# fpthink/PDGN

Measured on AMD Instinct MI355X. Metric: generator+D step points/sec (B=35, 256->2048 pts), higher is better.
Workload: dtype f32; 1 GPU; PDGNet_v2 G+D iteration (models/PDGNet_v2.py:171-256), chair-shaped synthetic batch, per-GPU batch 35, 256->2048 pts, random-init weights; global_batch=35, parallelism=dp1, losses_finite=True, hipgraph=False, issue=list

## Files before the change

include/pdgn_hip.h:

```cpp
#ifndef PDGN_HIP_H
#define PDGN_HIP_H

#include <stdint.h>

#ifdef __cplusplus
extern "C" {
#endif

#define PDGN_ERR_INVALID (-1)
#define PDGN_KNN_MAX_NSAMPLE 200

typedef void *pdgn_stream_t;

#define PDGN_ABI_VERSION 34
int pdgn_abi_version(void);

int pdgn_knnquery(int b, int n, int m, int nsample, const float *xyz, const float *new_xyz,
                  int32_t *idx, float *dist2, pdgn_stream_t stream);

int pdgn_grouping_forward(int b, int c, int n, int m, int nsample, const float *points,
                          const int32_t *idx, float *out, pdgn_stream_t stream);

int pdgn_grouping_backward(int b, int c, int n, int m, int nsample, const float *grad_out,
                           const int32_t *idx, float *grad_points, pdgn_stream_t stream);

int pdgn_nearestneighbor(int b, int n, int m, const float *unknown, const float *known,
                         float *dist2, int32_t *idx, pdgn_stream_t stream);

int pdgn_interpolation_forward(int b, int c, int m, int n, const float *points,
                               const int32_t *idx, const float *weight, float *out,
                               pdgn_stream_t stream);

int pdgn_interpolation_backward(int b, int c, int n, int m, const float *grad_out,
                                const int32_t *idx, const float *weight, float *grad_points,
                                pdgn_stream_t stream);

int pdgn_nndistance(int b, int n, const float *xyz, int m, const float *xyz2, float *result,
                    int32_t *result_i, float *result2, int32_t *result2_i, pdgn_stream_t stream);

int pdgn_nndistance_grad(int b, int n, const float *xyz1, int m, const float *xyz2,
                         const float *grad_dist1, const int32_t *idx1, const float *grad_dist2,
                         const int32_t *idx2, float *grad_xyz1, float *grad_xyz2,
                         pdgn_stream_t stream);

int pdgn_approxmatch(int b, int n, int m, const float *xyz1, const float *xyz2, float *match,
                     float *temp, pdgn_stream_t stream);

int pdgn_matchcost(int b, int n, int m, const float *xyz1, const float *xyz2,
                   const float *match, float *out, pdgn_stream_t stream);

int pdgn_matchcost_grad(int b, int n, int m, const float *xyz1, const float *xyz2,
                        const float *match, float *grad1, float *grad2, pdgn_stream_t stream);

long long pdgn_emd_cost_temp_floats(long long pairs, int n, int m);
int pdgn_emd_cost(int b, int n, int m, const float *xyz1, const float *xyz2, float *temp,
                  float *out, pdgn_stream_t stream);

int pdgn_feature_knn(int b, int f, int n, int k, const float *x, float *sqnorm, int32_t *idx,
                     pdgn_stream_t stream);

int pdgn_window_gather_sum(int b, int n, int k, int ldy, int T, int P, int C, int off, int offc,
                           const float *Y, const int32_t *idx, const float *bias, int bias_bstride,
                           float *out, pdgn_stream_t stream);
int pdgn_window_gather_sum_stats(int b, int n, int k, int ldy, int T, int P, int C, int off, int offc,
                                 const float *Y, const int32_t *idx, const float *bias, int bias_bstride,
                                 float *out, float *scratch, pdgn_stream_t stream);

int pdgn_window_gather_sum_backward(int b, int n, int k, int ldy, int T, int P, int C, int off,
                                    int offc, const float *dout, const int32_t *idx, float *dY,
                                    pdgn_stream_t stream);

int pdgn_knn_graph_transpose(int b, int n, int k, const int32_t *idx, int32_t *rowptr, int32_t *edges,
                             int32_t *scratch, pdgn_stream_t stream);
int pdgn_window_gather_sum_backward_csr(int b, int n, int k, int ldy, int T, int P, int C, int off,
                                        int offc, const float *dout, const int32_t *rowptr,
                                        const int32_t *edges, float *dY, unsigned *max_out, int max_init, pdgn_stream_t stream);

long long pdgn_bn_scratch_floats(long long rows, int c);
int pdgn_bn_stats(long long rows, int c, float eps, float momentum, const float *x, const float *gamma,
                  const float *beta, const float *pre_bias, float *running_mean, float *running_var,
                  float *scratch, float *stats, pdgn_stream_t stream);
int pdgn_bn_eval_stats(int c, float eps, const float *gamma, const float *beta, const float *pre_bias,
                       const float *running_mean, const float *running_var, float *stats,
                       pdgn_stream_t stream);
int pdgn_bn_stats_from_partials(long long rows, int c, float eps, float momentum, const float *gamma,
                                const float *beta, const float *pre_bias, float *running_mean, float *running_var,
                                const float *scratch, float *stats, pdgn_stream_t stream);
int pdgn_bn_stats_from_gemm_partials(long long rows, int c, long long nparts, int block_rows, float eps, float momentum,
                                     const float *gamma, const float *beta, const float *pre_bias,
                                     float *running_mean, float *running_var, const float *partials,
                                     float *stats, double *scratch, pdgn_stream_t stream);
long long pdgn_bn_blocks_scratch_doubles(int c, long long nparts);
int pdgn_bn_act_forward(long long rows, int c, int act, const float *x, const float *stats,
                        const float *mul, float *y, int interleave_n, pdgn_stream_t stream);
int pdgn_bn_act_backward(long long rows, int c, int act, int training, const float *x,
                         const float *dy, const float *mul, const float *stats, float *scratch,
                         float *bsums, float *dx, float *dmul, int interleave_n, pdgn_stream_t stream);

long long pdgn_bn_maxpool_scratch_floats(int b, int c);
int pdgn_bn_act_maxpool(int b, int n, int c, int act, const float *x, const float *stats, float *scratch,
                        float *ymax, int32_t *yarg, pdgn_stream_t stream);
long long pdgn_bn_stats_maxpool_scratch_floats(int b, int c);
int pdgn_bn_stats_act_maxpool(int b, int n, int c, int act, float eps, float momentum, const float *x, const float *gamma,
                              const float *beta, const float *pre_bias, float *running_mean, float *running_var, float *scratch,
                              float *stats, float *ymax, int32_t *yarg, pdgn_stream_t stream);
int pdgn_bn_act_maxpool_backward(int b, int n, int c, int act, int training, const float *x,
                                 const float *dout, const int32_t *yarg, const float *stats,
                                 float *scratch, float *bsums, float *dx, pdgn_stream_t stream);
long long pdgn_dense_bn_maxpool_backward_scratch(int b, int c, int k);
int pdgn_dense_bn_maxpool_backward(int b, int n, int c, int k, int act, const float *x, const float *dout, const int32_t *yarg,
                                   const float *stats, const float *h, int ldh, const float *W, int ldw, float *scratch,
                                   float *dh, float *dW, int lddw, float *bsums, pdgn_stream_t stream);
long long pdgn_dense_bn_maxpool_input_grad_scratch(int b, int c, int k);
int pdgn_dense_bn_maxpool_input_grad(int b, int n, int c, int k, int act, const float *x, const float *dout,
                                     const int32_t *yarg, const float *stats, const float *h, int ldh,
                                     const float *W, int ldw, float *scratch, float *dh, pdgn_stream_t stream);

int pdgn_group_colsum(long long groups, long long group_rows, int c, const float *x, long long ldx, float *out,
                      pdgn_stream_t stream);

int pdgn_softmax_slots_permute(long long m, int k, int c, const float *h, float *w, pdgn_stream_t stream);
int pdgn_bn_softmax_slots_permute(long long m, int k, int c, int act, const float *x, const float *stats,
                                  float *w, pdgn_stream_t stream);
int pdgn_bn_softmax_slots_permute_mul(long long m, int k, int c, int act, const float *x, const float *stats,
                                      int act_u, const float *u, const float *stats_u, float *w, float *y,
                                      unsigned *max_out, const float *gamma_u, const float *beta_u, float bound_scale,
                                      unsigned *cmax_out, pdgn_stream_t stream);
long long pdgn_bilateral_scratch_floats(long long m, int k, int c);
int pdgn_bilateral_weighting_backward(long long m, int k, int c, int act, int training, const float *x,
                                      const float *stats_x, const float *u, const float *stats_u, const float *w,
                                      const float *dy, float *scratch, float *bsums_x, float *bsums_u, float *dx,
                                      float *du, pdgn_stream_t stream);
int pdgn_softmax_slots_permute_backward(long long m, int k, int c, const float *w, const float *dw,
                                        float *dh, pdgn_stream_t stream);

int pdgn_skinny_nt(int R, int N, int K, const float *A, int lda, const float *B, int ldb, const float *bias, float *C, int ldc,
                   pdgn_stream_t stream);
int pdgn_skinny_nn(int R, int N, int K, const float *A, int lda, const float *B, int ldb, float *C, int ldc, pdgn_stream_t stream);
int pdgn_skinny_nt_act(int R, int N, int K, const float *A, int lda, const float *B, int ldb, const float *bias, float *C, int ldc,
                       int act, pdgn_stream_t stream);
int pdgn_skinny_nn_masked(int R, int N, int K, const float *A, int lda, const float *P, int ldp, int act, const float *B,
                          int ldb, float *C, int ldc, pdgn_stream_t stream);
int pdgn_skinny_tn(int R, int N, int K, const float *A, int lda, const float *B, int ldb, float *C, int ldc, pdgn_stream_t stream);
int pdgn_split_bf16x3(int rows, int cols, const float *src, int ld_src, unsigned short *planes, int ld_planes,
                      long long plane_stride, unsigned short *planes_t, int ld_planes_t, long long plane_stride_t,
                      pdgn_stream_t stream);
int pdgn_gemm_nt_ps(long long m, int n, int k, const float *A, int lda, const unsigned short *Wplanes, int ldw, long long wplane,
                    int parts, const float *bias, const float *addend, int ldadd, float *C, int ldc, float *stat_part,
                    const float *row_bias, int ld_rb, int rows_per_group, int act, const float *gate, int ldgate,
                    pdgn_stream_t stream);
long long pdgn_gemm_tail_workspace_floats(long long m, int n, int k, int with_stats);
long long pdgn_gemm_tn_big_workspace_floats(long long m, int n, int k);
int pdgn_gemm_set_tail_workspace(float *ws, long long floats);
int pdgn_gemm_nt_ps_launch_info(long long m, int n, int k, int parts, const void **sym, int *grid);
int pdgn_gemm_aux_symbols(const void **reduce, const void **scan);
int pdgn_gemm_set_mode(int mode);
int pdgn_gemm_set_scale_slots(void *slots, long long bytes);
int pdgn_absmax_rows_cols(long long rows, int cols, const float *src, int ld, unsigned *rowmax, unsigned *colmax,
                          pdgn_stream_t stream);
int pdgn_gemm_set_operand_scales(const unsigned *max_a, const unsigned *max_w);
int pdgn_gemm_two_part(long long m, int n, int k, long long scan_bytes);
int pdgn_gemm_two_part_planes(long long m, int n, int k, long long scan_bytes);
long long pdgn_gemm_nt_ps_stat_rows(long long m, int n, int k, int parts, int plain);
int pdgn_gemm_nt_ps_stat_block_rows(long long m, int n, int k, int parts, int plain);
int pdgn_gemm_nt_ps_row_panel(long long m, int n, int k, int parts, int plain);
long long pdgn_gemm_nt_ps_workspace_floats(long long m, int n, int k, int parts, int with_stats);
int pdgn_split_f16x2(int rows, int cols, const float *src, int ld_src, unsigned short *planes, int ld_planes,
                     long long plane_stride, unsigned short *planes_t, int ld_planes_t, long long plane_stride_t,
                     pdgn_stream_t stream);
int pdgn_gemm_set_config(int cfg);
int pdgn_gemm_set_shape(int shape);
int pdgn_gemm_nt(long long m, int n, int k, const float *A, int lda, const float *W, int ldw,
                 const float *bias, const float *addend, int ldadd, float *C, int ldc, float *stat_part,
                 pdgn_stream_t stream);
long long pdgn_thin_stat_rows(long long m);
int pdgn_thin_stat_block_rows(void);
int pdgn_thin_nt(long long m, int n, int k, const float *X, int ldx, const float *W, int wrs, int wcs,
                 const float *bias, float *Y, int ldy, float *stat_part, pdgn_stream_t stream);
int pdgn_thin_nt_ex(long long m, int n, int k, const float *X, int ldx, const float *W, int wrs, int wcs,
                    const float *bias, float *Y, int ldy, float *stat_part, const float *gate, int ldgate, pdgn_stream_t stream);
int pdgn_thin_tn(long long m, int ta, int wb, const float *A, int lda, const float *B, int ldb, float *O, int osi,
                 int osj, float *sum_a, float *sum_b, pdgn_stream_t stream);
int pdgn_gemm_nn(long long m, int n, int k, const float *A, int lda, const float *Wt, int ldw,
                 const float *bias, const float *addend, int ldadd, float *C, int ldc, float *stat_part,
                 pdgn_stream_t stream);
int pdgn_gemm_tn_big(long long m, int n, int k, const float *dY, int ldy, const float *X, int ldx, float *dW, int dw_is_zero,
                     pdgn_stream_t stream);
int pdgn_gemm_nt_ex(long long m, int n, int k, const float *A, int lda, const float *W, int ldw, const float *bias,
                    const float *addend, int ldadd, float *C, int ldc, float *stat_part, const float *row_bias, int ld_rb,
                    int rows_per_group, int act, const float *gate, int ldgate, int transposed_w, pdgn_stream_t stream);
long long pdgn_gemm_nt_stat_rows(long long m, int n, int k);
int pdgn_gemm_nt_stat_block_rows(long long m, int n, int k);
int pdgn_gemm_nt_config(long long m, int n, int k, int with_stats);

int pdgn_gemm_tn(long long m, int n, int k, const float *dY, const float *X, float *dW,
                 pdgn_stream_t stream);

int pdgn_local_stats(int b, int n, int m, int k, const float *xyz, const int32_t *idx, float *mu,
                     float *cov, pdgn_stream_t stream);
int pdgn_local_stats_backward(int b, int n, int m, int k, const float *xyz, const int32_t *idx,
                              const float *dmu, const float *dcov, float *dxyz, pdgn_stream_t stream);

int pdgn_chamfer_gram(int b, int m, int n, int d, const float *x, const float *y, float *minx,
                      int32_t *argx, float *miny, int32_t *argy, pdgn_stream_t stream);
int pdgn_chamfer_gram_grad(int b, int m, int n, int d, const float *x, const float *y,
                           const float *gminx, const int32_t *argx, const float *gminy,
                           const int32_t *argy, float *gx, float *gy, pdgn_stream_t stream);
int pdgn_chamfer_gram_grad_uniform(int b, int m, int n, int d, const float *x, const float *y, const float *g,
                                   float scale, const int32_t *argx, const int32_t *argy, float *gx, float *gy,
                                   pdgn_stream_t stream);
int pdgn_scaled_sum(long long n, const float *x, float scale, float *out, pdgn_stream_t stream);
int pdgn_mse_const(long long n, const float *x, float target, float scale, float *out, pdgn_stream_t stream);
int pdgn_mse_const_backward(long long n, const float *x, float target, float scale, const float *g, float *dx,
                            pdgn_stream_t stream);

int pdgn_emd_cost_indexed(int npairs, int n, int m, const float *xyz1, const int32_t *ia,
                          const float *xyz2, const int32_t *ib, float *temp, float *out,
                          pdgn_stream_t stream);
int pdgn_chamfer_gram_indexed(int npairs, int m, int n, int d, const float *x, const int32_t *ia,
                              const float *y, const int32_t *ib, float *minx, int32_t *argx,
                              float *miny, int32_t *argy, pdgn_stream_t stream);

int pdgn_deconv_assemble(int F, int Fo, int k, int T, int fc, const float *Wi, const float *W2, const float *Wf,
                         float *WcatC, float *WcatV, float *Wb, pdgn_stream_t stream);
int pdgn_deconv_assemble_backward(int F, int Fo, int k, int T, int fc, const float *gWcatC, const float *gWcatV,
                                  const float *gWb, float *dWi, float *dW2, float *dWf, pdgn_stream_t stream);

int pdgn_sample_bias(int b, int ldy, int nspec, const int *T, const int *C, const int *off, const int *offc,
                     const float *const *bias, const float *Yc, float *bb, pdgn_stream_t stream);
int pdgn_sample_bias_backward(int b, int ldy, int nspec, const int *T, const int *C, const int *off, const int *offc,
                              const float *g, float *dYc, float *const *dbias, pdgn_stream_t stream);

int pdgn_small_mlp_forward(int r, int k, int n, int act, int bn_mode, float eps, float momentum, const float *x,
                           const float *W, const float *bias, const float *gamma, const float *beta,
                           float *running_mean, float *running_var, float *y, float *pre, float *stat,
                           pdgn_stream_t stream);
int pdgn_small_mlp_backward(int r, int k, int n, int act, int bn_mode, const float *x, const float *dy, const float *pre,
                            const float *stat, const float *gamma, const float *beta, float *dpre, float *dgamma,
                            float *dbeta, float *dbias, float *dW, pdgn_stream_t stream);

int pdgn_ballquery(int b, int n, int m, float radius, int nsample, const float *new_xyz, const float *xyz,
                   int32_t *idx, pdgn_stream_t stream);
int pdgn_furthestsampling(int b, int n, int m, const float *xyz, float *temp, int32_t *idx, pdgn_stream_t stream);
int pdgn_gathering_forward(int b, int c, int n, int m, const float *points, const int32_t *idx, float *out,
                           pdgn_stream_t stream);
int pdgn_gathering_backward(int b, int c, int n, int m, const float *grad_out, const int32_t *idx,
                            float *grad_points, pdgn_stream_t stream);
int pdgn_grouping_int_forward(int b, int c, int n, int m, int nsample, const long long *points, const int32_t *idx,
                              long long *out, pdgn_stream_t stream);
int pdgn_featuredistribute(int b, int n, int m, const float *max_xyz, const float *xyz, int32_t *distribute_idx,
                           pdgn_stream_t stream);
int pdgn_labelstat_idx(int b, int n, int m, int nsample, int nclass, const int32_t *label_stat, const int32_t *idx,
                       int32_t *new_label_stat, pdgn_stream_t stream);
int pdgn_labelstat_ballrange(int b, int n, int m, float radius, int nclass, const float *new_xyz, const float *xyz,
                             const int32_t *label_stat, int32_t *new_label_stat, pdgn_stream_t stream);
int pdgn_labelstat_and_ballquery(int b, int n, int m, float radius, int nsample, int nclass, const float *new_xyz,
                                 const float *xyz, const int32_t *label_stat, int32_t *idx, int32_t *new_label_stat,
                                 pdgn_stream_t stream);

long long pdgn_point_max_scratch(int b, int n, int c);
int pdgn_point_max(int b, int n, int c, const float *x, float *scratch_val, int32_t *scratch_arg, float *out, int32_t *arg,
                   pdgn_stream_t stream);
int pdgn_point_max_backward(int b, int n, int c, const float *grad_out, const int32_t *arg, float *grad_x,
                            pdgn_stream_t stream);

int pdgn_spin(unsigned int microseconds, pdgn_stream_t stream);

int pdgn_replay_marker(int id, pdgn_stream_t stream);
int pdgn_replay_build(void *hip_graph, void **plan_out);
int pdgn_replay_info(void *plan, int *counts8);
int pdgn_replay_chains(void *plan, int *labels, int *nodes_per_chain);
int pdgn_replay_set_stream(void *plan, int chain, pdgn_stream_t stream);
int pdgn_replay_launch(void *plan);
int pdgn_replay_launch_range(void *plan, int lo, int hi);
int pdgn_replay_position(void *plan, int chain, int nth);
int pdgn_replay_points(void *plan, int *ids, int *pos, int *chain, int max_out);
int pdgn_replay_joined(void *plan);
int pdgn_replay_kernel_nodes(void *plan, const void *sym, int gx, int *pos, int max_out);
int pdgn_replay_chain_neighbor(void *plan, int pos, int dir, int *kind_out, const void **sym_out);
int pdgn_replay_time_spans(void *plan, const int *first, const int *last, int n, int slots);
int pdgn_replay_time_read(void *plan, float *ms_out, int *counts);
int pdgn_replay_launch_timed(void *plan, double *us32);
int pdgn_replay_probe_chain(void *plan, int chain, int stride, float *ms_out, int *pos_out, int max_out);
int pdgn_replay_destroy(void *plan);

int pdgn_adam_multi(int ntensors, void *const *p, const void *const *g, void *const *m, void *const *v, const long long *n, double lr,
                    double beta1, double beta2, double eps, const float *step, pdgn_stream_t stream);
int pdgn_copy_multi(int ntensors, void *const *dst, const void *const *src, const long long *n, pdgn_stream_t stream);
int pdgn_adam_ema_multi(int ntensors, void *const *p, const void *const *g, void *const *m, void *const *v, void *const *e,
                        const long long *n, double lr, double beta1, double beta2, double eps, double ema_decay, const float *step,
                        pdgn_stream_t stream);
int pdgn_ema_multi(int ntensors, void *const *e, const void *const *p, const long long *n, double ema_decay, const float *step,
                   pdgn_stream_t stream);

typedef struct pdgn_guard_record {
    float norm;
    float coef;
    float applied;
    float found_inf;
    unsigned n_applied;
    unsigned n_skipped;
    unsigned reserved[2];
} pdgn_guard_record;
long long pdgn_gradnorm_workspace_doubles(int ntensors, const long long *n);
int pdgn_gradnorm_multi(int ntensors, const void *const *g, const long long *n, double max_norm, double *workspace,
                        long long workspace_doubles, pdgn_guard_record *record, pdgn_stream_t stream);
int pdgn_adam_guard_multi(int ntensors, void *const *p, const void *const *g, void *const *m, void *const *v, const long long *n,
                          double lr, double beta1, double beta2, double eps, const float *step, const pdgn_guard_record *guard,
                          pdgn_stream_t stream);
int pdgn_adam_ema_guard_multi(int ntensors, void *const *p, const void *const *g, void *const *m, void *const *v, void *const *e,
                              const long long *n, double lr, double beta1, double beta2, double eps, double ema_decay, const float *step,
                              const pdgn_guard_record *guard, pdgn_stream_t stream);
int pdgn_ema_guard_multi(int ntensors, void *const *e, const void *const *p, const long long *n, double ema_decay, const float *step,
                         const pdgn_guard_record *guard, pdgn_stream_t stream);

#define PDGN_LR_MAX_KNOTS 16
#define PDGN_LR_TABLE_DOUBLES 33
int pdgn_adam_sched_multi(int ntensors, void *const *p, const void *const *g, void *const *m, void *const *v, void *const *e,
                          const long long *n, double lr, double beta1, double beta2, double eps, double ema_decay, const float *step,
                          const pdgn_guard_record *guard, const double *sched, pdgn_stream_t stream);
int pdgn_lr_eval(const double *sched, double lr, const float *step, const pdgn_guard_record *guard, double *out2, float *out_lr32,
                 pdgn_stream_t stream);

int pdgn_set_deterministic(int on);
long long pdgn_det_workspace_ints(int b, int targets, long long edges);
int pdgn_grouping_backward_det(int b, int c, int n, int m, int nsample, const float *grad_out, const int32_t *idx,
                               int32_t *ws, float *grad_points, pdgn_stream_t stream);
int pdgn_interpolation_backward_det(int b, int c, int n, int m, const float *grad_out, const int32_t *idx,
                                    const float *weight, int32_t *ws, float *grad_points, pdgn_stream_t stream);
int pdgn_gathering_backward_det(int b, int c, int n, int m, const float *grad_out, const int32_t *idx, int32_t *ws,
                                float *grad_points, pdgn_stream_t stream);
int pdgn_nndistance_grad_det(int b, int n, const float *xyz1, int m, const float *xyz2, const float *grad_dist1,
                             const int32_t *idx1, const float *grad_dist2, const int32_t *idx2, int32_t *ws,
                             float *grad_xyz1, float *grad_xyz2, pdgn_stream_t stream);

int pdgn_feed_batch(int B, int S, int N, int r1, int r2, int r3, const float *data, const int32_t *order, long long first,
                    unsigned long long seed, unsigned long long t, long long row0, float sigma, float *p1, float *p2, float *p3,
                    float *p4, float *z1, float *z2, pdgn_stream_t stream);

int pdgn_feed_batch_resample(int B, int S, int M, int P, int N, int r1, int r2, int r3, const float *data, const int32_t *order,
                             long long first, unsigned long long seed, unsigned long long t, long long row0, float sigma, float *p1,
                             float *p2, float *p3, float *p4, float *z1, float *z2, pdgn_stream_t stream);

typedef struct pdgn_aug_table {
    unsigned thr_flip, thr_rot, thr_scale, thr_trans, thr_jitter;
    int flip_axis, up_axis;
    float rot_max;
    float log_scale_max;
    float trans_max;
    float sigma;
    unsigned reserved[5];
} pdgn_aug_table;
#define PDGN_AUG_TAG_BASE 16
#define PDGN_AUG_SITES 12
int pdgn_augment_rows_fwd(int B, int N, const float *x, int x_point_major, float *rows, float *affine_out, const pdgn_aug_table *table,
                          const unsigned long long *clock, unsigned long long seed, long long row0, int tag, pdgn_stream_t stream);
int pdgn_augment_rows_bwd(int B, int N, const float *d_rows, float *dx, int dx_point_major, const pdgn_aug_table *table,
                          const unsigned long long *clock, unsigned long long seed, long long row0, int tag, pdgn_stream_t stream);
int pdgn_augment_tick(unsigned long long *clock, pdgn_stream_t stream);

long long pdgn_render_workspace_bytes(int rows, int cols, int cell);
int pdgn_render_sheet(int rows, int cols, const float *const *clouds, const int *npoints, int channel_major, const float *view,
                      int cell, int radius, void *workspace, uint8_t *image, pdgn_stream_t stream);

#ifdef __cplusplus
}
#endif
#endif
```

pdgn_amd/csrc/knn3.hip:

```cpp
#include "common.h"
#include "wave_select.h"

#define KNN_THREADS 256
#define KNN_WAVES (KNN_THREADS / PDGN_WAVE)
#define KNN_TILE 4096
#define KNN_FAST_MAX_K 32


#define KNN4_THREADS 512
#define KNN4_WAVES (KNN4_THREADS / PDGN_WAVE)
#define KNN4_Q 2
#define KNN4_TILE 2048
#define KNN4_QCAP 64

__device__ __forceinline__ float wave_kth_smallest_ub16(float v, int K) {
    const unsigned key = __float_as_uint(v) | 0x80000000u;
    unsigned prefix = 0x80000000u;
#pragma unroll
    for (int bit = 30; bit >= 15; --bit) {
        const unsigned cand = prefix | (1u << bit);
        const int below = __popcll(__ballot(key < cand));
        prefix = below < K ? cand : prefix;
    }
    const unsigned ub = min(prefix | 0x7fffu, 0xff800000u);
    return __uint_as_float(ub & 0x7fffffffu);
}

__global__ __launch_bounds__(KNN4_THREADS) void knn3_wave4_kernel(
    int n, int m, int K, int qpw, const float *__restrict__ xyz, const float *__restrict__ new_xyz,
    int32_t *__restrict__ idx, float *__restrict__ dist2) {
    __shared__ float4 cand[KNN4_TILE];
    __shared__ DI queue[KNN4_WAVES][KNN4_Q][KNN4_QCAP + KNN_FAST_MAX_K];
    __shared__ DI win[KNN4_WAVES][KNN4_Q][KNN_FAST_MAX_K];

    const int bs = blockIdx.y;
    const int lane = lane_id();
    const int wave = threadIdx.x / PDGN_WAVE;
    const float *P = xyz + (size_t)bs * n * 3;
  for (int grp = 0; grp < qpw; ++grp) {
    const int q0 = ((blockIdx.x * KNN4_WAVES + wave) * qpw + grp) * KNN4_Q;

    float qx[KNN4_Q], qy[KNN4_Q], qz[KNN4_Q], rd[KNN4_Q];
    int ri[KNN4_Q], cnt[KNN4_Q];
#pragma unroll
    for (int q = 0; q < KNN4_Q; ++q) {
        const int query = min(q0 + q, m - 1);
        const float *Qp = new_xyz + ((size_t)bs * m + query) * 3;
        qx[q] = Qp[0]; qy[q] = Qp[1]; qz[q] = Qp[2];
        rd[q] = INFINITY;
        ri[q] = 0x7fffffff;
        cnt[q] = 0;
    }
    const bool vec_ok = (n % 4 == 0) && ((reinterpret_cast<uintptr_t>(xyz) & 15) == 0);
    for (int t0 = 0; t0 < n; t0 += KNN4_TILE) {
        const int tn = min(KNN4_TILE, n - t0);
        const int tp = (tn + 255) & ~255;
      if (grp == 0 || n > KNN4_TILE) {
        __syncthreads();
        if (vec_ok) {
            const float4 *src = reinterpret_cast<const float4 *>(P + (size_t)t0 * 3);
            for (int g = threadIdx.x; g < tn / 4; g += KNN4_THREADS) {
                const float4 a = src[3 * g], b = src[3 * g + 1], c = src[3 * g + 2];
                cand[4 * g] = make_float4(a.x, a.y, a.z, 0.f);
                cand[4 * g + 1] = make_float4(a.w, b.x, b.y, 0.f);
                cand[4 * g + 2] = make_float4(b.z, b.w, c.x, 0.f);
                cand[4 * g + 3] = make_float4(c.y, c.z, c.w, 0.f);
            }
        } else {
            for (int c = threadIdx.x; c < tn; c += KNN4_THREADS) {
                const float *pp = P + (size_t)(t0 + c) * 3;
                cand[c] = make_float4(pp[0], pp[1], pp[2], 0.f);
            }
        }
        for (int c = tn + threadIdx.x; c < tp; c += KNN4_THREADS) cand[c] = make_float4(INFINITY, INFINITY, INFINITY, 0.f);
        __syncthreads();
      }
        float lmin[KNN4_Q];
#pragma unroll
        for (int q = 0; q < KNN4_Q; ++q) lmin[q] = INFINITY;
        for (int c = lane; c < tp; c += 256) {
            float4 p[4];
#pragma unroll
            for (int j = 0; j < 4; ++j) p[j] = cand[c + 64 * j];
#pragma unroll
            for (int j = 0; j < 4; ++j)
#pragma unroll
                for (int q = 0; q < KNN4_Q; ++q) {
                    const float d = sqdist3(qx[q], qy[q], qz[q], p[j].x, p[j].y, p[j].z);
                    lmin[q] = d < lmin[q] ? d : lmin[q];
                }
        }
        float tau[KNN4_Q];
        {
            unsigned key[KNN4_Q], prefix[KNN4_Q];
#pragma unroll
            for (int q = 0; q < KNN4_Q; ++q) { key[q] = __float_as_uint(lmin[q]) | 0x80000000u; prefix[q] = 0x80000000u; }
#pragma unroll
            for (int bit = 30; bit >= 15; --bit) {
                unsigned long long lo[KNN4_Q];
#pragma unroll
                for (int q = 0; q < KNN4_Q; ++q) lo[q] = __ballot(key[q] < (prefix[q] | (1u << bit)));
#pragma unroll
                for (int q = 0; q < KNN4_Q; ++q)
                    prefix[q] = __builtin_amdgcn_readfirstlane(__popcll(lo[q]) < K ? (prefix[q] | (1u << bit)) : prefix[q]);
            }
#pragma unroll
            for (int q = 0; q < KNN4_Q; ++q) {
                const unsigned ub = min(prefix[q] | 0x7fffu, 0xff800000u);
                tau[q] = fminf(__uint_as_float(ub & 0x7fffffffu), __shfl(rd[q], K - 1, 64));
            }
        }
#pragma unroll
        for (int q = 0; q < KNN4_Q; ++q) tau[q] = fminf(tau[q], 3.402823466e38f);
        int sc[KNN4_Q];
#pragma unroll
        for (int q = 0; q < KNN4_Q; ++q) sc[q] = __builtin_amdgcn_readfirstlane(cnt[q]);
        for (int c0 = 0; c0 < tp; c0 += 128) {
            float4 p[2];
#pragma unroll
            for (int j = 0; j < 2; ++j) p[j] = cand[c0 + 64 * j + lane];
#pragma unroll
            for (int j = 0; j < 2; ++j) {
                const int c = c0 + 64 * j + lane;
                float d[KNN4_Q];
                unsigned long long mask[KNN4_Q];
                int add[KNN4_Q];
                bool over = false;
#pragma unroll
                for (int q = 0; q < KNN4_Q; ++q) {
                    d[q] = sqdist3(qx[q], qy[q], qz[q], p[j].x, p[j].y, p[j].z);
                    mask[q] = __ballot(d[q] <= tau[q]);
                }
#pragma unroll
                for (int q = 0; q < KNN4_Q; ++q) {
                    add[q] = __popcll(mask[q]);
                    over = over || sc[q] + add[q] > KNN4_QCAP;
                }
                if (!over) {
#pragma unroll
                    for (int q = 0; q < KNN4_Q; ++q) {
                        const int pos = __builtin_amdgcn_mbcnt_hi((unsigned)(mask[q] >> 32), __builtin_amdgcn_mbcnt_lo((unsigned)mask[q], sc[q]));
                        if (d[q] <= tau[q]) { queue[wave][q][pos].d = d[q]; queue[wave][q][pos].i = t0 + c; }
                        sc[q] += add[q];
                    }
                } else {
#pragma unroll
                    for (int q = 0; q < KNN4_Q; ++q) {
                        DI *qq = queue[wave][q];
                        bool keep = d[q] <= tau[q];
                        unsigned long long mk = mask[q];
                        if (sc[q] + add[q] > KNN4_QCAP) {
                            knn_flush_ranked(qq, sc[q], K, rd[q], ri[q], lane, win[wave][q]);
                            sc[q] = 0;
                            tau[q] = fminf(tau[q], __shfl(rd[q], K - 1, 64));
                            keep = keep && d[q] <= tau[q];
                            mk = __ballot(keep);
                        }
                        const int pos = sc[q] + __popcll(mk & ((1ull << lane) - 1ull));
                        if (keep) { qq[pos].d = d[q]; qq[pos].i = t0 + c; }
                        sc[q] = __builtin_amdgcn_readfirstlane(sc[q] + __popcll(mk));
                    }
                }
            }
        }
        {
            DI *const qs[KNN4_Q] = {queue[wave][0], queue[wave][1]};
            knn_flush_select_multi<KNN4_Q>(qs, sc, K, rd, ri, lane, win[wave][0]);
        }
#pragma unroll
        for (int q = 0; q < KNN4_Q; ++q) cnt[q] = 0;
    }
#pragma unroll
    for (int q = 0; q < KNN4_Q; ++q) {
        const int query = q0 + q;
        if (query < m && lane < K) {
            const size_t o = ((size_t)bs * m + query) * K + lane;
            const bool valid = rd[q] < INFINITY;
            idx[o] = valid ? ri[q] : 0;
            if (dist2) dist2[o] = rd[q];
        }
    }
  }
}

__global__ __launch_bounds__(KNN_THREADS) void knn3_generic_kernel(
    int n, int m, int K, const float *__restrict__ xyz, const float *__restrict__ new_xyz,
    int32_t *__restrict__ idx, float *__restrict__ dist2) {
    const int bs = blockIdx.y;
    const int query = blockIdx.x * blockDim.x + threadIdx.x;
    if (query >= m) return;
    const float *P = xyz + (size_t)bs * n * 3;
    const float *Q = new_xyz + ((size_t)bs * m + query) * 3;
    const float qx = Q[0], qy = Q[1], qz = Q[2];
    float best[PDGN_KNN_MAX_NSAMPLE];
    int besti[PDGN_KNN_MAX_NSAMPLE];
    for (int i = 0; i < K; ++i) { best[i] = INFINITY; besti[i] = 0; }
    for (int c = 0; c < n; ++c) {
        float d = sqdist3(qx, qy, qz, P[c * 3], P[c * 3 + 1], P[c * 3 + 2]);
        if (d < best[K - 1]) {
            int j = K - 1;
            while (j > 0 && d < best[j - 1]) { best[j] = best[j - 1]; besti[j] = besti[j - 1]; --j; }
            best[j] = d;
            besti[j] = c;
        }
    }
    size_t o = ((size_t)bs * m + query) * K;
    for (int i = 0; i < K; ++i) {
        idx[o + i] = besti[i];
        if (dist2) dist2[o + i] = best[i];
    }
}

__global__ __launch_bounds__(KNN_THREADS) void nn3_kernel(
    int n, int m, const float *__restrict__ unknown, const float *__restrict__ known,
    float *__restrict__ dist2, int32_t *__restrict__ idx) {
    __shared__ float4 cand[2048];
    const int bs = blockIdx.y;
    const int j = blockIdx.x * blockDim.x + threadIdx.x;
    const float *Kn = known + (size_t)bs * m * 3;
    float ux = 0.f, uy = 0.f, uz = 0.f;
    if (j < n) {
        const float *U = unknown + ((size_t)bs * n + j) * 3;
        ux = U[0]; uy = U[1]; uz = U[2];
    }
    float b1 = INFINITY, b2 = INFINITY, b3 = INFINITY;
    int i1 = 0, i2 = 0, i3 = 0;
    for (int t0 = 0; t0 < m; t0 += 2048) {
        const int tn = min(2048, m - t0);
        __syncthreads();
        for (int e = threadIdx.x; e < tn * 3; e += KNN_THREADS)
            reinterpret_cast<float *>(cand)[(e / 3) * 4 + (e % 3)] = Kn[(size_t)t0 * 3 + e];
        __syncthreads();
        for (int c = 0; c < tn; ++c) {
            float4 p = cand[c];
            float d = sqdist3(ux, uy, uz, p.x, p.y, p.z);
            int k = t0 + c;
            if (d < b1) { b3 = b2; i3 = i2; b2 = b1; i2 = i1; b1 = d; i1 = k; }
            else if (d < b2) { b3 = b2; i3 = i2; b2 = d; i2 = k; }
            else if (d < b3) { b3 = d; i3 = k; }
        }
    }
    if (j < n) {
        size_t o = ((size_t)bs * n + j) * 3;
        dist2[o] = b1; dist2[o + 1] = b2; dist2[o + 2] = b3;
        idx[o] = i1; idx[o + 1] = i2; idx[o + 2] = i3;
    }
}

extern "C" int pdgn_knnquery(int b, int n, int m, int nsample, const float *xyz,
                             const float *new_xyz, int32_t *idx, float *dist2,
                             pdgn_stream_t stream) {
    if (b < 0 || n < 0 || m < 0 || nsample < 1 || nsample > PDGN_KNN_MAX_NSAMPLE) return PDGN_ERR_INVALID;
    if (b == 0 || m == 0) return 0;
    if (b > 65535) return PDGN_ERR_INVALID;
    hipStream_t s = (hipStream_t)stream;
    if (nsample <= KNN_FAST_MAX_K) {
        dim3 grid(cdiv(m, KNN4_WAVES * KNN4_Q), b);
        hipLaunchKernelGGL(knn3_wave4_kernel, grid, dim3(KNN4_THREADS), 0, s, n, m, nsample, 1, xyz, new_xyz, idx, dist2);
    } else {
        dim3 grid(cdiv(m, KNN_THREADS), b);
        hipLaunchKernelGGL(knn3_generic_kernel, grid, dim3(KNN_THREADS), 0, s, n, m, nsample, xyz,
                           new_xyz, idx, dist2);
    }
    return pdgn_launch_status();
}

extern "C" int pdgn_nearestneighbor(int b, int n, int m, const float *unknown, const float *known,
                                    float *dist2, int32_t *idx, pdgn_stream_t stream) {
    if (b < 0 || n < 0 || m < 0 || b > 65535) return PDGN_ERR_INVALID;
    if (b == 0 || n == 0) return 0;
    dim3 grid(cdiv(n, KNN_THREADS), b);
    hipLaunchKernelGGL(nn3_kernel, grid, dim3(KNN_THREADS), 0, (hipStream_t)stream, n, m, unknown,
                       known, dist2, idx);
    return pdgn_launch_status();
}
```

pdgn_amd/csrc/localpair.hip:

```cpp
#include "common.h"
#include <stdlib.h>

#define LP_THREADS 256
#define LP_LDS_FLOATS 8192
#define LP_PTS_FLOATS 6144

__global__ __launch_bounds__(LP_THREADS) void local_stats_fwd_kernel(
    int n, int m, int K, const float *__restrict__ xyz, const int32_t *__restrict__ idx,
    float *__restrict__ mu, float *__restrict__ cov) {
    const int bs = blockIdx.y;
    const int q = blockIdx.x * blockDim.x + threadIdx.x;
    if (q >= m) return;
    const float *P = xyz + (size_t)bs * n * 3;
    const int32_t *I = idx + ((size_t)bs * m + q) * K;
    float sx = 0.f, sy = 0.f, sz = 0.f;
    for (int s = 0; s < K; ++s) {
        const float *p = P + (size_t)I[s] * 3;
        sx += p[0]; sy += p[1]; sz += p[2];
    }
    const float invK = 1.0f / (float)K;
    const float mx = sx * invK, my = sy * invK, mz = sz * invK;
    float c00 = 0.f, c01 = 0.f, c02 = 0.f, c11 = 0.f, c12 = 0.f, c22 = 0.f;
    for (int s = 0; s < K; ++s) {
        const float *p = P + (size_t)I[s] * 3;
        const float tx = p[0] - mx, ty = p[1] - my, tz = p[2] - mz;
        c00 = __fmaf_rn(tx, tx, c00); c01 = __fmaf_rn(tx, ty, c01); c02 = __fmaf_rn(tx, tz, c02);
        c11 = __fmaf_rn(ty, ty, c11); c12 = __fmaf_rn(ty, tz, c12); c22 = __fmaf_rn(tz, tz, c22);
    }
    float *M = mu + ((size_t)bs * m + q) * 3;
    M[0] = mx; M[1] = my; M[2] = mz;
    float *C = cov + ((size_t)bs * m + q) * 9;
    C[0] = c00 * invK; C[1] = c01 * invK; C[2] = c02 * invK;
    C[3] = c01 * invK; C[4] = c11 * invK; C[5] = c12 * invK;
    C[6] = c02 * invK; C[7] = c12 * invK; C[8] = c22 * invK;
}

__global__ __launch_bounds__(LP_THREADS) void local_stats_bwd_kernel(
    int n, int m, int K, int qsplit, const float *__restrict__ xyz, const int32_t *__restrict__ idx,
    const float *__restrict__ dmu, const float *__restrict__ dcov, float *__restrict__ dxyz) {
    __shared__ float slab[LP_LDS_FLOATS];
    __shared__ float pts[LP_PTS_FLOATS];
    const int bs = blockIdx.y;
    const bool use_lds = n * 3 <= LP_LDS_FLOATS, use_pts = n * 3 <= LP_PTS_FLOATS;
    const float *P = xyz + (size_t)bs * n * 3;
    if (use_lds)
        for (int i = threadIdx.x; i < n * 3; i += LP_THREADS) slab[i] = 0.f;
    if (use_pts)
        for (int i = threadIdx.x; i < n * 3; i += LP_THREADS) pts[i] = P[i];
    if (use_lds || use_pts) __syncthreads();
    auto pt = [&](int j, int c) { return use_pts ? pts[j * 3 + c] : P[(size_t)j * 3 + c]; };
    float *D = dxyz + (size_t)bs * n * 3;
    const int per = (m + qsplit - 1) / qsplit;
    const int q0 = blockIdx.x * per, q1 = min(m, q0 + per);
    const float invK = 1.0f / (float)K;
    for (int q = q0 + threadIdx.x; q < q1; q += LP_THREADS) {
        const int32_t *I = idx + ((size_t)bs * m + q) * K;
        float sx = 0.f, sy = 0.f, sz = 0.f;
        for (int s = 0; s < K; ++s) {
            const int j = I[s];
            sx += pt(j, 0); sy += pt(j, 1); sz += pt(j, 2);
        }
        const float mx = sx * invK, my = sy * invK, mz = sz * invK;
        const float *gm = dmu + ((size_t)bs * m + q) * 3;
        const float *G = dcov + ((size_t)bs * m + q) * 9;
        const float s00 = 2.f * G[0], s01 = G[1] + G[3], s02 = G[2] + G[6];
        const float s11 = 2.f * G[4], s12 = G[5] + G[7], s22 = 2.f * G[8];
        const float bx = gm[0] * invK, by = gm[1] * invK, bz = gm[2] * invK;
        for (int s = 0; s < K; ++s) {
            const int j = I[s];
            const float tx = pt(j, 0) - mx, ty = pt(j, 1) - my, tz = pt(j, 2) - mz;
            const float gx = bx + (s00 * tx + s01 * ty + s02 * tz) * invK;
            const float gy = by + (s01 * tx + s11 * ty + s12 * tz) * invK;
            const float gz = bz + (s02 * tx + s12 * ty + s22 * tz) * invK;
            float *dst = use_lds ? &slab[j * 3] : &D[(size_t)j * 3];
            atomicAdd(dst, gx); atomicAdd(dst + 1, gy); atomicAdd(dst + 2, gz);
        }
    }
    if (use_lds) {
        __syncthreads();
        for (int i = threadIdx.x; i < n * 3; i += LP_THREADS) {
            float v = slab[i];
            if (v != 0.f) atomicAdd(&D[i], v);
        }
    }
}

#define CH_MAXD 16
#define CH_TILE 1024

template <int D>
__global__ __launch_bounds__(LP_THREADS) void chamfer_gram_kernel(
    int m, int n, int dd, const float *__restrict__ x, const float *__restrict__ y,
    float *__restrict__ minx, int32_t *__restrict__ argx, float *__restrict__ miny,
    int32_t *__restrict__ argy, const int32_t *__restrict__ ia, const int32_t *__restrict__ ib) {
    constexpr int DS = D > 0 ? D : CH_MAXD;
    __shared__ float cand[CH_TILE * (DS + 1)];
    const int d = D > 0 ? D : dd;
    const int bs = blockIdx.y;
    const bool rev = blockIdx.z != 0;
    const int nq = rev ? n : m, nc = rev ? m : n;
    if ((int)(blockIdx.x * blockDim.x) >= nq) return;
    const size_t bx = ia ? (size_t)ia[bs] : (size_t)bs, by = ib ? (size_t)ib[bs] : (size_t)bs;
    const float *Q = rev ? y + by * nq * d : x + bx * nq * d;
    const float *C = rev ? x + bx * nc * d : y + by * nc * d;
    const int i = blockIdx.x * blockDim.x + threadIdx.x;
    float qv[DS];
    float rq = 0.f;
#pragma unroll
    for (int c = 0; c < DS; ++c) {
        qv[c] = (c < d && i < nq) ? Q[(size_t)i * d + c] : 0.f;
        rq = __fmaf_rn(qv[c], qv[c], rq);
    }
    float best = INFINITY;
    int best_j = 0;
    for (int t0 = 0; t0 < nc; t0 += CH_TILE) {
        const int tn = min(CH_TILE, nc - t0);
        __syncthreads();
        for (int j = threadIdx.x; j < tn; j += LP_THREADS) {
            float r = 0.f;
            for (int c = 0; c < d; ++c) {
                float v = C[(size_t)(t0 + j) * d + c];
                cand[j * (DS + 1) + c] = v;
                r = __fmaf_rn(v, v, r);
            }
            cand[j * (DS + 1) + DS] = r;
        }
        __syncthreads();
        for (int j = 0; j < tn; ++j) {
            const float *cv = &cand[j * (DS + 1)];
            float dot = 0.f;
#pragma unroll
            for (int c = 0; c < DS; ++c)
                if (c < d) dot = __fmaf_rn(qv[c], cv[c], dot);
            const float p = (rq + cv[DS]) - 2.0f * dot;
            const bool better = p < best;
            best = better ? p : best;
            best_j = better ? t0 + j : best_j;
        }
    }
    if (i < nq) {
        (rev ? miny : minx)[(size_t)bs * nq + i] = best;
        (rev ? argy : argx)[(size_t)bs * nq + i] = best_j;
    }
}

__global__ __launch_bounds__(LP_THREADS) void chamfer_gram_grad_kernel(
    int m, int n, int d, const float *__restrict__ x, const float *__restrict__ y,
    const float *__restrict__ gminx, const int32_t *__restrict__ argx, const float *__restrict__ gminy,
    const int32_t *__restrict__ argy, float *__restrict__ gx, float *__restrict__ gy, const float *__restrict__ guni, float gscale) {
    const int bs = blockIdx.y;
    const bool rev = blockIdx.z != 0;
    const int nq = rev ? n : m, nc = rev ? m : n;
    const int i = blockIdx.x * blockDim.x + threadIdx.x;
    if (i >= nq) return;
    const float *Q = (rev ? y : x) + ((size_t)bs * nq + i) * d;
    const int j = (rev ? argy : argx)[(size_t)bs * nq + i];
    const float *C = (rev ? x : y) + ((size_t)bs * nc + j) * d;
    const float g = 2.0f * (guni ? guni[0] * gscale : (rev ? gminy : gminx)[(size_t)bs * nq + i]);
    float *GQ = (rev ? gy : gx) + ((size_t)bs * nq + i) * d;
    float *GC = (rev ? gx : gy) + ((size_t)bs * nc + j) * d;
    for (int c = 0; c < d; ++c) {
        const float v = g * (Q[c] - C[c]);
        atomicAdd(&GQ[c], v);
        atomicAdd(&GC[c], -v);
    }
}

#define CHL_THREADS 1024
#define CHL_MAXF 12288
template <int D>
__global__ __launch_bounds__(CHL_THREADS) void chamfer_gram_grad_lds_kernel(
    int m, int n, int d, const float *__restrict__ x, const float *__restrict__ y,
    const float *__restrict__ gminx, const int32_t *__restrict__ argx, const float *__restrict__ gminy,
    const int32_t *__restrict__ argy, float *__restrict__ gx, float *__restrict__ gy, const float *__restrict__ guni, float gscale) {
    __shared__ float accs[CHL_MAXF];
    const int dd = D > 0 ? D : d;
    const int bs = blockIdx.y;
    const bool rev = blockIdx.z != 0;
    const int nq = rev ? n : m, nc = rev ? m : n;
    const float *Qb = (rev ? y : x) + (size_t)bs * nq * dd, *Cb = (rev ? x : y) + (size_t)bs * nc * dd;
    const int32_t *own_arg = (rev ? argy : argx) + (size_t)bs * nq, *oth_arg = (rev ? argx : argy) + (size_t)bs * nc;
    const float *own_g = (rev ? gminy : gminx) + (guni ? 0 : (size_t)bs * nq), *oth_g = (rev ? gminx : gminy) + (guni ? 0 : (size_t)bs * nc);
    const float uni = guni ? 2.0f * guni[0] * gscale : 0.f;
    for (int f = threadIdx.x; f < nq * dd; f += CHL_THREADS) {
        const int i = f / dd, c = f - i * dd;
        const float g = guni ? uni : 2.0f * own_g[i];
        accs[f] = g * (Qb[f] - Cb[(size_t)own_arg[i] * dd + c]);
    }
    __syncthreads();
    for (int f = threadIdx.x; f < nc * dd; f += CHL_THREADS) {
        const int e = f / dd, c = f - e * dd;
        const int tgt = oth_arg[e];
        const float ge = guni ? uni : 2.0f * oth_g[e];
        __hip_atomic_fetch_add(&accs[tgt * dd + c], ge * (Qb[(size_t)tgt * dd + c] - Cb[f]), __ATOMIC_RELAXED,
                               __HIP_MEMORY_SCOPE_WORKGROUP);
    }
    __syncthreads();
    float *G = (rev ? gy : gx) + (size_t)bs * nq * dd;
    for (int f = threadIdx.x; f < nq * dd; f += CHL_THREADS) G[f] = accs[f];
}

extern "C" int pdgn_local_stats(int b, int n, int m, int k, const float *xyz, const int32_t *idx, float *mu,
                                float *cov, pdgn_stream_t stream) {
    if (b < 0 || n < 1 || m < 0 || k < 1 || b > 65535) return PDGN_ERR_INVALID;
    if (b == 0 || m == 0) return 0;
    hipLaunchKernelGGL(local_stats_fwd_kernel, dim3(cdiv(m, LP_THREADS), b), dim3(LP_THREADS), 0,
                       (hipStream_t)stream, n, m, k, xyz, idx, mu, cov);
    return pdgn_launch_status();
}

extern "C" int pdgn_local_stats_backward(int b, int n, int m, int k, const float *xyz, const int32_t *idx,
                                         const float *dmu, const float *dcov, float *dxyz,
                                         pdgn_stream_t stream) {
    if (b < 0 || n < 1 || m < 0 || k < 1 || b > 65535) return PDGN_ERR_INVALID;
    if (b == 0 || m == 0) return 0;
    int qsplit = 1024 / b;
    const int max_split = cdiv(m, LP_THREADS);
    qsplit = qsplit < 1 ? 1 : (qsplit > max_split ? max_split : qsplit);
    hipLaunchKernelGGL(local_stats_bwd_kernel, dim3(qsplit, b), dim3(LP_THREADS), 0, (hipStream_t)stream, n, m, k,
                       qsplit, xyz, idx, dmu, dcov, dxyz);
    return pdgn_launch_status();
}

static int chamfer_launch(dim3 grid, hipStream_t s, int m, int n, int d, const float *x, const float *y, float *minx,
                          int32_t *argx, float *miny, int32_t *argy, const int32_t *ia, const int32_t *ib) {
    if (d == 3)
        hipLaunchKernelGGL(chamfer_gram_kernel<3>, grid, dim3(LP_THREADS), 0, s, m, n, d, x, y, minx, argx, miny, argy, ia, ib);
    else if (d == 9)
        hipLaunchKernelGGL(chamfer_gram_kernel<9>, grid, dim3(LP_THREADS), 0, s, m, n, d, x, y, minx, argx, miny, argy, ia, ib);
    else
        hipLaunchKernelGGL(chamfer_gram_kernel<0>, grid, dim3(LP_THREADS), 0, s, m, n, d, x, y, minx, argx, miny, argy, ia, ib);
    return pdgn_launch_status();
}

extern "C" int pdgn_chamfer_gram(int b, int m, int n, int d, const float *x, const float *y, float *minx,
                                 int32_t *argx, float *miny, int32_t *argy, pdgn_stream_t stream) {
    if (b < 0 || m < 1 || n < 1 || d < 1 || d > CH_MAXD || b > 65535) return PDGN_ERR_INVALID;
    if (b == 0) return 0;
    dim3 grid(cdiv(m > n ? m : n, LP_THREADS), b, 2);
    hipStream_t s = (hipStream_t)stream;
    return chamfer_launch(grid, s, m, n, d, x, y, minx, argx, miny, argy, nullptr, nullptr);
}

extern "C" int pdgn_chamfer_gram_indexed(int npairs, int m, int n, int d, const float *x, const int32_t *ia,
                                         const float *y, const int32_t *ib, float *minx, int32_t *argx,
                                         float *miny, int32_t *argy, pdgn_stream_t stream) {
    if (npairs < 0 || m < 1 || n < 1 || d < 1 || d > CH_MAXD || npairs > 65535) return PDGN_ERR_INVALID;
    if (npairs == 0) return 0;
    dim3 grid(cdiv(m > n ? m : n, LP_THREADS), npairs, 2);
    return chamfer_launch(grid, (hipStream_t)stream, m, n, d, x, y, minx, argx, miny, argy, ia, ib);
}

static int chamfer_grad_launch(int b, int m, int n, int d, const float *x, const float *y, const float *gminx, const int32_t *argx,
                               const float *gminy, const int32_t *argy, float *gx, float *gy, const float *guni, float gscale,
                               hipStream_t s) {
    hipError_t e;
    const size_t nx = (size_t)b * m * d, ny = (size_t)b * n * d;
    static const bool in_lds = !(getenv("PDGN_CHAMFER_LDS") && getenv("PDGN_CHAMFER_LDS")[0] == '0');
    if (in_lds && (size_t)m * d <= CHL_MAXF && (size_t)n * d <= CHL_MAXF) {
        dim3 grid(1, b, 2);
        if (d == 3)
            hipLaunchKernelGGL(chamfer_gram_grad_lds_kernel<3>, grid, dim3(CHL_THREADS), 0, s, m, n, d, x, y, gminx, argx, gminy, argy,
                               gx, gy, guni, gscale);
        else if (d == 9)
            hipLaunchKernelGGL(chamfer_gram_grad_lds_kernel<9>, grid, dim3(CHL_THREADS), 0, s, m, n, d, x, y, gminx, argx, gminy, argy,
                               gx, gy, guni, gscale);
        else
            hipLaunchKernelGGL(chamfer_gram_grad_lds_kernel<0>, grid, dim3(CHL_THREADS), 0, s, m, n, d, x, y, gminx, argx, gminy, argy,
                               gx, gy, guni, gscale);
        return pdgn_launch_status();
    }
    if (gy == gx + nx) {
        if ((e = hipMemsetAsync(gx, 0, (nx + ny) * sizeof(float), s)) != hipSuccess) return (int)e;
    } else {
        if ((e = hipMemsetAsync(gx, 0, nx * sizeof(float), s)) != hipSuccess) return (int)e;
        if ((e = hipMemsetAsync(gy, 0, ny * sizeof(float), s)) != hipSuccess) return (int)e;
    }
    dim3 grid(cdiv(m > n ? m : n, LP_THREADS), b, 2);
    hipLaunchKernelGGL(chamfer_gram_grad_kernel, grid, dim3(LP_THREADS), 0, s, m, n, d, x, y, gminx, argx, gminy, argy, gx, gy,
                       guni, gscale);
    return pdgn_launch_status();
}

extern "C" int pdgn_chamfer_gram_grad(int b, int m, int n, int d, const float *x, const float *y,
                                      const float *gminx, const int32_t *argx, const float *gminy,
                                      const int32_t *argy, float *gx, float *gy, pdgn_stream_t stream) {
    if (b < 0 || m < 1 || n < 1 || d < 1 || d > CH_MAXD || b > 65535) return PDGN_ERR_INVALID;
    if (b == 0) return 0;
    return chamfer_grad_launch(b, m, n, d, x, y, gminx, argx, gminy, argy, gx, gy, nullptr, 0.f, (hipStream_t)stream);
}

extern "C" int pdgn_chamfer_gram_grad_uniform(int b, int m, int n, int d, const float *x, const float *y, const float *g,
                                              float scale, const int32_t *argx, const int32_t *argy, float *gx, float *gy,
                                              pdgn_stream_t stream) {
    if (b < 0 || m < 1 || n < 1 || d < 1 || d > CH_MAXD || b > 65535 || !g) return PDGN_ERR_INVALID;
    if (b == 0) return 0;
    return chamfer_grad_launch(b, m, n, d, x, y, nullptr, argx, nullptr, argy, gx, gy, g, scale, (hipStream_t)stream);
}
```

pdgn_amd/csrc/loss_small.hip:

```cpp
#include "common.h"

#define LS_THREADS 1024

__device__ __forceinline__ float ls_block_sum(float v) {
    __shared__ float red[LS_THREADS / PDGN_WAVE];
#pragma unroll
    for (int off = 32; off > 0; off >>= 1) v += __shfl_xor(v, off, 64);
    if (lane_id() == 0) red[threadIdx.x / PDGN_WAVE] = v;
    __syncthreads();
    float s = 0.f;
    if (threadIdx.x == 0)
        for (int w = 0; w < LS_THREADS / PDGN_WAVE; ++w) s += red[w];
    return s;
}

__global__ __launch_bounds__(LS_THREADS) void scaled_sum_kernel(long long n, const float *__restrict__ x, float scale,
                                                               float *__restrict__ out) {
    float s = 0.f;
    for (long long i = threadIdx.x; i < n; i += LS_THREADS) s += x[i];
    s = ls_block_sum(s);
    if (threadIdx.x == 0) out[0] = scale * s;
}

__global__ __launch_bounds__(LS_THREADS) void mse_const_fwd_kernel(long long n, const float *__restrict__ x, float t, float scale,
                                                                  float *__restrict__ out) {
    float s = 0.f;
    for (long long i = threadIdx.x; i < n; i += LS_THREADS) {
        const float d = x[i] - t;
        s = __fmaf_rn(d, d, s);
    }
    s = ls_block_sum(s);
    if (threadIdx.x == 0) out[0] = scale * (s / (float)n);
}

__global__ __launch_bounds__(256) void mse_const_bwd_kernel(long long n, const float *__restrict__ x, float t, float scale,
                                                            const float *__restrict__ g, float *__restrict__ dx) {
    const float c = g[0] * scale * 2.0f / (float)n;
    for (long long i = (long long)blockIdx.x * blockDim.x + threadIdx.x; i < n; i += (long long)gridDim.x * blockDim.x)
        dx[i] = c * (x[i] - t);
}

extern "C" int pdgn_scaled_sum(long long n, const float *x, float scale, float *out, pdgn_stream_t stream) {
    if (n < 0) return PDGN_ERR_INVALID;
    hipLaunchKernelGGL(scaled_sum_kernel, dim3(1), dim3(LS_THREADS), 0, (hipStream_t)stream, n, x, scale, out);
    return pdgn_launch_status();
}

extern "C" int pdgn_mse_const(long long n, const float *x, float target, float scale, float *out, pdgn_stream_t stream) {
    if (n < 1) return PDGN_ERR_INVALID;
    hipLaunchKernelGGL(mse_const_fwd_kernel, dim3(1), dim3(LS_THREADS), 0, (hipStream_t)stream, n, x, target, scale, out);
    return pdgn_launch_status();
}

extern "C" int pdgn_mse_const_backward(long long n, const float *x, float target, float scale, const float *g, float *dx,
                                       pdgn_stream_t stream) {
    if (n < 1) return PDGN_ERR_INVALID;
    const int grid = (int)(n < 256 * 64 ? cdiv(n, 256) : 64);
    hipLaunchKernelGGL(mse_const_bwd_kernel, dim3(grid), dim3(256), 0, (hipStream_t)stream, n, x, target, scale, g, dx);
    return pdgn_launch_status();
}
```

pdgn_amd/losses.py:

```python

import torch
import torch.nn as nn
from ._fn import Function

from . import _lib, pointops
from ._lib import check, ptr, require, stream_of
from .fused import _zeros

F32, I32 = torch.float32, torch.int32


class ChamferGram(Function):

    @staticmethod
    def forward(ctx, x, y):
        x, y = x.contiguous(), y.contiguous()
        require(x, "x", F32, 3)
        require(y, "y", F32, 3)
        b, m, d = x.shape
        n = y.shape[1]
        minx = torch.empty((b, m), dtype=F32, device=x.device)
        miny = torch.empty((b, n), dtype=F32, device=x.device)
        argx = torch.empty((b, m), dtype=I32, device=x.device)
        argy = torch.empty((b, n), dtype=I32, device=x.device)
        check(_lib.lib().pdgn_chamfer_gram(b, m, n, d, ptr(x), ptr(y), ptr(minx), ptr(argx), ptr(miny), ptr(argy),
                                           stream_of(x)), "pdgn_chamfer_gram")
        ctx.save_for_backward(x, y, argx, argy)
        ctx.mark_non_differentiable(argx, argy)
        return minx, miny

    @staticmethod
    def backward(ctx, gminx, gminy):
        x, y, argx, argy = ctx.saved_tensors
        b, m, d = x.shape
        n = y.shape[1]
        gx, gy = torch.empty_like(x), torch.empty_like(y)
        gminx, gminy = gminx.contiguous(), gminy.contiguous()
        check(_lib.lib().pdgn_chamfer_gram_grad(b, m, n, d, ptr(x), ptr(y), ptr(gminx), ptr(argx), ptr(gminy),
                                                ptr(argy), ptr(gx), ptr(gy), stream_of(x)),
              "pdgn_chamfer_gram_grad")
        return gx, gy


def chamfer_min(x, y):
    return ChamferGram.apply(x, y)


class ChamferSum(Function):

    @staticmethod
    def forward(ctx, x, y, scale):
        x, y = x.contiguous(), y.contiguous()
        require(x, "x", F32, 3)
        require(y, "y", F32, 3)
        b, m, d = x.shape
        n = y.shape[1]
        mins = torch.empty((b * (m + n),), dtype=F32, device=x.device)
        args = torch.empty((b * (m + n),), dtype=I32, device=x.device)
        minx, miny, argx, argy = mins[:b * m], mins[b * m:], args[:b * m], args[b * m:]
        check(_lib.lib().pdgn_chamfer_gram(b, m, n, d, ptr(x), ptr(y), ptr(minx), ptr(argx), ptr(miny), ptr(argy),
                                           stream_of(x)), "pdgn_chamfer_gram")
        ctx.save_for_backward(x, y, args)
        ctx.scale = float(scale)
        out = torch.empty((), dtype=F32, device=x.device)
        check(_lib.lib().pdgn_scaled_sum(b * (m + n), ptr(mins), ctx.scale, ptr(out), stream_of(x)), "pdgn_scaled_sum")
        return out

    @staticmethod
    def backward(ctx, g):
        x, y, args = ctx.saved_tensors
        b, m, d = x.shape
        n = y.shape[1]
        gbuf = torch.empty((b * (m + n) * d,), dtype=F32, device=x.device)
        gx, gy = gbuf[:b * m * d].view(b, m, d), gbuf[b * m * d:].view(b, n, d)
        g = g.contiguous()
        check(_lib.lib().pdgn_chamfer_gram_grad_uniform(b, m, n, d, ptr(x), ptr(y), ptr(g), ctx.scale,
                                                        ptr(args[:b * m]), ptr(args[b * m:]), ptr(gx), ptr(gy), stream_of(x)),
              "pdgn_chamfer_gram_grad_uniform")
        return gx, gy, None


class MseConst(Function):

    @staticmethod
    def forward(ctx, x, target, scale):
        x = x.contiguous()
        require(x, "x", F32)
        out = torch.empty((), dtype=F32, device=x.device)
        check(_lib.lib().pdgn_mse_const(x.numel(), ptr(x), target, scale, ptr(out), stream_of(x)), "pdgn_mse_const")
        ctx.save_for_backward(x)
        ctx.cfg = (float(target), float(scale))
        return out

    @staticmethod
    def backward(ctx, g):
        x, = ctx.saved_tensors
        target, scale = ctx.cfg
        dx = torch.empty_like(x)
        g = g.contiguous()
        check(_lib.lib().pdgn_mse_const_backward(x.numel(), ptr(x), target, scale, ptr(g), ptr(dx), stream_of(x)), "pdgn_mse_const_backward")
        return dx, None, None


def mse_const(x, target, scale=1.0):
    return MseConst.apply(x, float(target), float(scale))


def chamfer_sum(x, y, scale=1.0):
    return ChamferSum.apply(x, y, scale)


class LocalStats(Function):

    @staticmethod
    def forward(ctx, xyz, idx):
        require(xyz, "xyz", F32, 3)
        require(idx, "idx", I32, 3)
        b, n, _ = xyz.shape
        _, m, k = idx.shape
        mu = torch.empty((b, m, 3), dtype=F32, device=xyz.device)
        cov = torch.empty((b, m, 9), dtype=F32, device=xyz.device)
        check(_lib.lib().pdgn_local_stats(b, n, m, k, ptr(xyz), ptr(idx), ptr(mu), ptr(cov), stream_of(xyz)),
              "pdgn_local_stats")
        ctx.save_for_backward(xyz, idx)
        return mu, cov

    @staticmethod
    def backward(ctx, dmu, dcov):
        xyz, idx = ctx.saved_tensors
        b, n, _ = xyz.shape
        _, m, k = idx.shape
        dxyz = _zeros(tuple(xyz.shape), xyz.device)
        dmu, dcov = dmu.contiguous(), dcov.contiguous()
        check(_lib.lib().pdgn_local_stats_backward(b, n, m, k, ptr(xyz), ptr(idx), ptr(dmu), ptr(dcov), ptr(dxyz),
                                                   stream_of(xyz)), "pdgn_local_stats_backward")
        return dxyz, None


def local_stats(xyz, idx):
    return LocalStats.apply(xyz, idx)


def knnquery(nsample, xyz, new_xyz):
    return pointops.knnquery(nsample, xyz, new_xyz)


class ChamferLoss(nn.Module):

    def forward(self, preds, gts):
        return chamfer_sum(gts, preds, 1.0)


def compute_mean_covariance(points):
    mu = points.mean(dim=-1, keepdim=True)
    tmp = points - mu
    return mu, torch.bmm(tmp, tmp.transpose(1, 2)) / points.shape[-1]


class LocalPairLoss(nn.Module):

    def __init__(self, nsample=20):
        super().__init__()
        self.nsample = nsample
        self.chamfer_loss = ChamferLoss()

    def stats(self, cloud_cl, query_cl):
        idx = knnquery(self.nsample, cloud_cl, query_cl)
        return local_stats(cloud_cl, idx)

    def forward(self, pt1, pt2, self_stats=None):
        M = pt1.shape[2]
        new_xyz = pt1.transpose(1, 2).contiguous()
        mu1, var1 = self_stats if self_stats is not None else self.stats(new_xyz, new_xyz)
        mu2, var2 = self.stats(pt2.transpose(1, 2).contiguous(), new_xyz)
        return chamfer_sum(mu2, mu1, 1.0 / float(M)), chamfer_sum(var2, var1, 1.0 / float(M))
```

pdgn_amd/trainer.py:

```python
import contextlib
import ctypes
import os
import warnings

import torch
import torch.distributed as dist
import torch.nn as nn

from . import _lib
from . import schedule as _schedule
from . import streams as _streams
from .fused import clear_zero_colsum, flush_bn_counters, hold_bn_counters, release_zero_arena, reset_zero_arena
from .generator import PointDiscriminator, PointGenerator
from . import losses
from .losses import LocalPairLoss

PAIRS = ((0, 1), (0, 2), (0, 3), (1, 2), (1, 3), (2, 3))


def _fp32_lists(*lists):
    first = lists[0]
    return bool(first) and first[0].is_cuda and all(
        len(lst) == len(first) and all(t.dtype == torch.float32 and t.is_contiguous() and t.device == f.device and t.numel() == f.numel()
                                       for t, f in zip(lst, first)) for lst in lists)


def _pointer_table(tensors):
    return (ctypes.c_void_p * len(tensors))(*[t.data_ptr() for t in tensors])


def _count_table(tensors):
    return (ctypes.c_longlong * len(tensors))(*[t.numel() for t in tensors])


class FlatGrads:

    def __init__(self, params, first=None):
        ps = [p for p in params if p.requires_grad]
        early = {id(p) for p in (first or [])}
        self.params = [p for p in ps if id(p) in early] + [p for p in ps if id(p) not in early]
        self.n_early = sum(1 for p in ps if id(p) in early)
        slot = lambda p: (p.numel() + 3) // 4 * 4
        total = sum(slot(p) for p in self.params)
        ref = self.params[0]
        self.buf = torch.zeros(total, dtype=ref.dtype, device=ref.device)
        self.views, off = [], 0
        for i, p in enumerate(self.params):
            if i == self.n_early:
                self.early_numel = off
            self.views.append(self.buf[off:off + p.numel()].view_as(p))
            off += slot(p)
        if self.n_early == len(self.params):
            self.early_numel = off
        self._early_work, self._early_done = None, False
        self._armed, self._arrived, self._hooks, self._group = False, 0, [], None

    def begin(self):
        for p in self.params:
            p.grad = None
        self._early_work, self._early_done = None, False
        self._arrived = 0
        clear_zero_colsum()
        if self.params and self.params[0].is_cuda:
            reset_zero_arena(self.params[0].device, self)

    def resume(self):
        if self.params and self.params[0].is_cuda:
            reset_zero_arena(self.params[0].device, self)

    def zero_(self):
        self.buf.zero_()

    def pack(self):
        self._pack(self.n_early if self._early_done else 0, len(self.params))

    def _pack(self, lo, hi):
        views, params = self.views[lo:hi], self.params[lo:hi]
        have = [(v, p) for v, p in zip(views, params) if p.grad is not None]
        missing = [v for v, p in zip(views, params) if p.grad is None]
        if have:
            self._copy([v for v, _ in have], [p.grad for _, p in have], (lo, hi) if len(have) == hi - lo else None)
        for v in missing:
            v.zero_()
        for v, p in zip(views, params):
            p.grad = v

    def _copy(self, dsts, srcs, full=None):
        if os.environ.get("PDGN_OWN_ADAM", "1") == "1" and _fp32_lists(dsts, srcs):
            cache = self.__dict__.setdefault("_copy_cache", {})
            hit = cache.get(full) if full is not None else None
            if hit is None:
                hit = (_pointer_table(dsts), _count_table(dsts))
                if full is not None:
                    cache[full] = hit
            _lib.check(_lib.lib().pdgn_copy_multi(len(dsts), hit[0], _pointer_table(srcs), hit[1], _lib.stream_of(dsts[0])), "pdgn_copy_multi")
            return
        torch._foreach_copy_(dsts, srcs)

    def arm_early(self, on=True, group=None):
        self._armed, self._group = bool(on), group
        if on and not self._hooks and self.n_early:
            for p in self.params[:self.n_early]:
                self._hooks.append(p.register_post_accumulate_grad_hook(self._arrival))

    def _arrival(self, _param):
        if not self._armed or self._early_done:
            return
        self._arrived += 1
        if self._arrived == self.n_early:
            self.reduce_early(self._group)

    def reduce_early(self, group=None):
        if self._early_done or self.n_early == 0 or not (dist.is_available() and dist.is_initialized()):
            return
        rec = _recorder(self.buf.device)
        if _capturing(self.buf.device) and rec is None:
            return
        if any(p.grad is None for p in self.params[:self.n_early]):
            return
        self._pack(0, self.n_early)
        self._early_done = True
        if rec is not None:

            def start(fg=self, group=group):
                fg._early_work = dist.all_reduce(fg.buf[:fg.early_numel], op=dist.ReduceOp.SUM, group=group, async_op=True)
            rec.point(start)
            return
        self._early_work = dist.all_reduce(self.buf[:self.early_numel], op=dist.ReduceOp.SUM, group=group, async_op=True)

    def all_reduce_mean(self, group=None):
        if dist.is_available() and dist.is_initialized():
            rec = _recorder(self.buf.device)
            if rec is not None:
                early = self._early_done

                def reduce(fg=self, group=group, early=early):
                    if early:
                        if fg.early_numel < fg.buf.numel():
                            dist.all_reduce(fg.buf[fg.early_numel:], op=dist.ReduceOp.SUM, group=group)
                        fg._early_work.wait()
                        fg._early_work = None
                    else:
                        dist.all_reduce(fg.buf, op=dist.ReduceOp.SUM, group=group)
                rec.point(reduce)
                if dist.get_world_size(group) > 1:
                    self.buf.div_(dist.get_world_size(group))
                return
            if self._early_done:
                if self.early_numel < self.buf.numel():
                    dist.all_reduce(self.buf[self.early_numel:], op=dist.ReduceOp.SUM, group=group)
                self._early_work.wait()
                self._early_work = None
            else:
                dist.all_reduce(self.buf, op=dist.ReduceOp.SUM, group=group)
            if dist.get_world_size(group) > 1:
                self.buf.div_(dist.get_world_size(group))


def _capturing(device):
    return device.type == "cuda" and torch.cuda.is_available() and torch.cuda.is_current_stream_capturing()


def _recorder(device):
    if device.type != "cuda":
        return None
    from . import replay
    rec = replay.recorder()
    return rec if rec is not None and _capturing(device) else None


class DeterminismWarning(UserWarning):
    """The library's deterministic mode is on, but the operation at hand has no fixed-order form yet."""


def _warn_if_deterministic(what):
    if _lib.deterministic():
        warnings.warn("PDGNTrainer.%s: deterministic mode is on, but the training step has no fixed-order form yet -- its "
                      "weight gradients and adjoints still sum with float atomics, so runs are not bitwise repeatable "
                      "(DESIGN.md section 5)" % what, DeterminismWarning, stacklevel=3)


def world_size():
    return dist.get_world_size() if dist.is_available() and dist.is_initialized() else 1


GUARD_RECORD_FLOATS = 8


class GradGuardError(RuntimeError):
    """`fit` saw `guard_max_skips` consecutive skipped updates of a network: its gradients have stopped being finite."""


class GradGuard:

    def __init__(self, params, max_norm=None, record=None):
        params = list(params)
        dev = params[0].device
        self.max_norm = 0.0 if max_norm is None else float(max_norm)
        if self.max_norm != self.max_norm or self.max_norm < 0:
            raise ValueError("clip_grad_norm must be a positive number (or None), got %r" % (max_norm,))
        self.record = record if record is not None else torch.zeros(GUARD_RECORD_FLOATS, dtype=torch.float32, device=dev)
        if (self.record.dtype != torch.float32 or self.record.numel() != GUARD_RECORD_FLOATS or not self.record.is_contiguous()
                or self.record.device != dev):
            raise ValueError("guard record: %d contiguous fp32 words on the parameters' device" % GUARD_RECORD_FLOATS)
        self.coef, self.applied, self.found_inf = self.record[1], self.record[2], self.record[3]
        self.counters = self.record.view(torch.int32)[4:6]
        counts = _count_table(params)
        self.workspace = torch.zeros(sum((p.numel() + 4095) // 4096 for p in params), dtype=torch.float64, device=dev)
        self._n, self._counts = len(params), counts

    def measure(self, grads):
        if len(grads) != self._n or not _fp32_lists(grads) or any(g.numel() != c for g, c in zip(grads, self._counts)):
            raise _lib.PdgnHipError("the gradient guard reads one contiguous fp32 gradient per parameter on a ROCm device; this list "
                                    "cannot be guarded")
        _lib.check(_lib.lib().pdgn_gradnorm_multi(self._n, _pointer_table(grads), self._counts, self.max_norm, _lib.ptr(self.workspace),
                                                  self.workspace.numel(), _lib.ptr(self.record), _lib.stream_of(grads[0])),
                   "pdgn_gradnorm_multi")

    @staticmethod
    def decode(words):
        ints = words.contiguous().view(torch.int32)
        return {"norm": float(words[0]), "coef": float(words[1]), "applied": int(ints[4]) & 0xffffffff, "skipped": int(ints[5]) & 0xffffffff}

    def state(self):
        return self.decode(self.record.cpu())


class LeanAdamStep:

    def __init__(self, opt, ema=None, ema_decay=0.0, guard=None, sched=None):
        self.opt, self.lists, self._table = opt, None, None
        self.ema, self.ema_decay, self._ema_table = (list(ema) if ema else None), float(ema_decay), None
        self.guard = guard
        self.sched = sched
        if sched is not None:
            if not (torch.is_tensor(sched) and sched.dtype == torch.float64 and sched.numel() == _schedule.TABLE_DOUBLES
                    and sched.is_contiguous()):
                raise ValueError("lr schedule: a contiguous torch.float64 tensor of %d words (schedule.table)" % _schedule.TABLE_DOUBLES)
            self.lr_out = torch.zeros(2, dtype=torch.float64, device=sched.device)
            self.lr32 = torch.zeros((), dtype=torch.float32, device=sched.device)

    def reset(self):
        self.lists = None
        self._table = None
        self._ema_table = None

    def _plain_step(self, measured=False):
        if self.guard is not None:
            self._guarded_plain_step(measured)
            return
        if self.sched is not None:
            self._scheduled_opt_step()
        else:
            self.opt.step()
        self._ema_alone()

    def _eval_lr(self, step=None):
        opt = self.opt
        if len(opt.param_groups) != 1 or not all(g.get("fused") and g.get("capturable") for g in opt.param_groups):
            raise _lib.PdgnHipError("a learning-rate schedule reaches torch's Adam as a tensor `lr`, which takes a fused, capturable "
                                    "optimizer with one parameter group; the unscheduled rate is not an option")
        g = opt.param_groups[0]
        if isinstance(g["lr"], torch.Tensor):
            raise _lib.PdgnHipError("a learning-rate schedule multiplies a Python float base rate; this group's lr is a tensor")
        if step is None:
            st = opt.state.get(g["params"][0])
            step = st["step"] if st and "step" in st else torch.zeros(1, dtype=torch.float32, device=self.sched.device)
        if not (torch.is_tensor(step) and step.is_cuda and step.dtype == torch.float32 and step.device == self.sched.device):
            raise _lib.PdgnHipError("a learning-rate schedule reads Adam's step count on the device: a capturable optimizer on the "
                                    "table's device is required")
        _lib.check(_lib.lib().pdgn_lr_eval(_lib.ptr(self.sched), float(g["lr"]), _lib.ptr(step),
                                           _lib.ptr(self.guard.record) if self.guard is not None else None, _lib.ptr(self.lr_out),
                                           _lib.ptr(self.lr32), _lib.stream_of(self.sched)), "pdgn_lr_eval")
        return self.lr32

    def _scheduled_opt_step(self):
        g = self.opt.param_groups[0] if self.opt.param_groups else None
        lr32 = self._eval_lr()
        base = g["lr"]
        g["lr"] = lr32
        try:
            self.opt.step()
        finally:
            g["lr"] = base

    def _guarded_plain_step(self, measured):
        opt, guard = self.opt, self.guard
        if len(opt.param_groups) != 1 or not all(g.get("fused") and g.get("capturable") for g in opt.param_groups):
            raise _lib.PdgnHipError("the gradient guard hands its skip flag to torch's fused, capturable Adam as `found_inf`; this "
                                    "optimizer cannot take it, and an unguarded update is not an option")
        params = opt.param_groups[0]["params"]
        if any(p.grad is None for p in params):
            raise _lib.PdgnHipError("the gradient guard needs a gradient for every parameter of the optimizer")
        if not measured:
            grads = [p.grad for p in params]
            guard.measure(grads)
            with torch.no_grad():
                torch._foreach_mul_(grads, guard.coef)
        opt.grad_scale, opt.found_inf = None, guard.found_inf
        try:
            if self.sched is not None:
                self._scheduled_opt_step()
            else:
                opt.step()
        finally:
            opt.grad_scale = opt.found_inf = None
        self._ema_alone()

    def _ema_alone(self):
        if self.ema is None:
            return
        ps = self.opt.param_groups[0]["params"]
        step = self.opt.state[ps[0]]["step"]
        n = len(ps)
        tab = self._ema_table
        if tab is None or tab[0] != n or tab[2][0] != ps[0].data_ptr() or tab[2][n - 1] != ps[n - 1].data_ptr():
            if not _fp32_lists(ps, self.ema):
                raise _lib.PdgnHipError("the averaged generator needs contiguous fp32 parameters on a ROCm device (pdgn_amd has no CPU path)")
            tab = self._ema_table = (n, _pointer_table(self.ema), _pointer_table(ps), _count_table(ps))
        if not (torch.is_tensor(step) and step.is_cuda and step.dtype == torch.float32):
            raise _lib.PdgnHipError("the averaged generator reads Adam's step count on the device: a capturable optimizer is required")
        if self.guard is not None:
            _lib.check(_lib.lib().pdgn_ema_guard_multi(n, tab[1], tab[2], tab[3], self.ema_decay, _lib.ptr(step), _lib.ptr(self.guard.record),
                                                       _lib.stream_of(ps[0])), "pdgn_ema_guard_multi")
            return
        _lib.check(_lib.lib().pdgn_ema_multi(n, tab[1], tab[2], tab[3], self.ema_decay, _lib.ptr(step), _lib.stream_of(ps[0])), "pdgn_ema_multi")

    _OWN = os.environ.get("PDGN_OWN_ADAM", "1") == "1"

    def _own_adam(self, ps, grads, exp_avgs, exp_avg_sqs, steps, g, launch=True):
        if not self._OWN or not ps or not ps[0].is_cuda:
            return False
        n = len(ps)
        tab = self._table
        if tab is None or tab[0] != n or tab[1][0] != ps[0].data_ptr() or tab[2][n - 1] != exp_avgs[n - 1].data_ptr():
            if not _fp32_lists(ps, exp_avgs, exp_avg_sqs) or steps[0].dtype != torch.float32:
                return False
            tab = self._table = (n, _pointer_table(ps), _pointer_table(exp_avgs), _pointer_table(exp_avg_sqs), _count_table(ps))
        if any(t.dtype != torch.float32 or not t.is_contiguous() for t in grads):
            return False
        et = None
        if self.ema is not None:
            et = self._ema_table
            if et is None or et[0] != n or et[2][0] != tab[1][0] or et[2][n - 1] != tab[1][n - 1]:
                return False
        if not launch:
            return True
        if self.sched is not None:
            _lib.check(_lib.lib().pdgn_adam_sched_multi(n, tab[1], _pointer_table(grads), tab[2], tab[3], et[1] if et is not None else None,
                                                        tab[4], g["lr"], g["betas"][0], g["betas"][1], g["eps"], self.ema_decay,
                                                        _lib.ptr(steps[0]), _lib.ptr(self.guard.record) if self.guard is not None else None,
                                                        _lib.ptr(self.sched), _lib.stream_of(ps[0])), "pdgn_adam_sched_multi")
            return True
        if self.ema is not None:
            if self.guard is not None:
                _lib.check(_lib.lib().pdgn_adam_ema_guard_multi(n, tab[1], _pointer_table(grads), tab[2], tab[3], et[1], tab[4], g["lr"],
                                                                g["betas"][0], g["betas"][1], g["eps"], self.ema_decay, _lib.ptr(steps[0]),
                                                                _lib.ptr(self.guard.record), _lib.stream_of(ps[0])), "pdgn_adam_ema_guard_multi")
                return True
            _lib.check(_lib.lib().pdgn_adam_ema_multi(n, tab[1], _pointer_table(grads), tab[2], tab[3], et[1], tab[4], g["lr"], g["betas"][0],
                                                      g["betas"][1], g["eps"], self.ema_decay, _lib.ptr(steps[0]), _lib.stream_of(ps[0])),
                       "pdgn_adam_ema_multi")
            return True
        if self.guard is not None:
            _lib.check(_lib.lib().pdgn_adam_guard_multi(n, tab[1], _pointer_table(grads), tab[2], tab[3], tab[4], g["lr"], g["betas"][0],
                                                        g["betas"][1], g["eps"], _lib.ptr(steps[0]), _lib.ptr(self.guard.record),
                                                        _lib.stream_of(ps[0])), "pdgn_adam_guard_multi")
            return True
        _lib.check(_lib.lib().pdgn_adam_multi(n, tab[1], _pointer_table(grads), tab[2], tab[3], tab[4], g["lr"], g["betas"][0], g["betas"][1],
                                              g["eps"], _lib.ptr(steps[0]), _lib.stream_of(ps[0])), "pdgn_adam_multi")
        return True

    def step(self):
        opt = self.opt
        if self.lists is None:
            self._plain_step()
            g = opt.param_groups[0]
            ok = (len(opt.param_groups) == 1 and g.get("fused") and g.get("capturable") and not g.get("amsgrad")
                  and not g.get("maximize") and not g.get("differentiable") and g.get("weight_decay", 0) == 0
                  and not isinstance(g["lr"], torch.Tensor) and all(p.grad is not None for p in g["params"])
                  and os.environ.get("PDGN_LEAN_ADAM", "1") == "1")
            if ok:
                ps, st = list(g["params"]), opt.state
                self.lists = (ps, [st[p]["exp_avg"] for p in ps], [st[p]["exp_avg_sq"] for p in ps], [st[p]["step"] for p in ps])
            else:
                self.lists = False
            return
        if self.lists is False:
            self._plain_step()
            return
        ps, exp_avgs, exp_avg_sqs, steps = self.lists
        grads = [p.grad for p in ps]
        g = opt.param_groups[0]
        st0 = opt.state.get(ps[0]) if ps else None
        if (len(opt.param_groups) != 1 or len(g["params"]) != len(ps) or g.get("weight_decay", 0) != 0 or g.get("amsgrad")
                or g.get("maximize") or isinstance(g["lr"], torch.Tensor) or st0 is None or st0.get("exp_avg") is not exp_avgs[0]
                or opt._optimizer_step_pre_hooks or opt._optimizer_step_post_hooks or any(gr is None for gr in grads)):
            self.lists = None
            self._plain_step()
            return
        if self.guard is not None:
            self._guarded_lean_step(ps, grads, exp_avgs, exp_avg_sqs, steps, g)
            return
        lr = g["lr"]
        if self.sched is not None and not self._own_adam(ps, grads, exp_avgs, exp_avg_sqs, steps, g, launch=False):
            lr = self._eval_lr(steps[0])
        try:
            with torch.no_grad():
                torch._foreach_add_(steps, 1)
                if self._own_adam(ps, grads, exp_avgs, exp_avg_sqs, steps, g):
                    return
                torch._fused_adam_(ps, grads, exp_avgs, exp_avg_sqs, [], steps, amsgrad=False, lr=lr, beta1=g["betas"][0],
                                   beta2=g["betas"][1], weight_decay=0.0, eps=g["eps"], maximize=False, grad_scale=None,
                                   found_inf=None)
                self._ema_alone()
        except TypeError:
            torch._foreach_sub_(steps, 1)
            self.lists = False
            self._plain_step()

    def _guarded_lean_step(self, ps, grads, exp_avgs, exp_avg_sqs, steps, g):
        guard = self.guard
        guard.measure(grads)
        scaled = False
        lr = g["lr"]
        if self.sched is not None and not self._own_adam(ps, grads, exp_avgs, exp_avg_sqs, steps, g, launch=False):
            lr = self._eval_lr(steps[0])
        try:
            with torch.no_grad():
                torch._foreach_add_(steps, [guard.applied] * len(steps))
                if self._own_adam(ps, grads, exp_avgs, exp_avg_sqs, steps, g):
                    return
                torch._foreach_mul_(grads, guard.coef)
                scaled = True
                torch._fused_adam_(ps, grads, exp_avgs, exp_avg_sqs, [], steps, amsgrad=False, lr=lr, beta1=g["betas"][0],
                                   beta2=g["betas"][1], weight_decay=0.0, eps=g["eps"], maximize=False, grad_scale=None,
                                   found_inf=guard.found_inf)
                self._ema_alone()
        except TypeError:
            torch._foreach_sub_(steps, [guard.applied] * len(steps))
            self.lists = False
            self._plain_step(measured=scaled)


class PDGNTrainer:

    def __init__(self, device="cuda", lr=1e-4, num_k=20, base_points=128, generator=None,
                 discriminators=None, distributed=None, ema_decay=0.0, grad_guard=False, clip_grad_norm=None,
                 lr_g=None, lr_d=None, lr_schedule=None, augment=None):
        if not 0.0 <= float(ema_decay) < 1.0:
            raise ValueError("ema_decay must be in [0, 1), got %r" % (ema_decay,))
        self.ema_decay = float(ema_decay)
        if clip_grad_norm is not None and not float(clip_grad_norm) > 0.0:
            raise ValueError("clip_grad_norm must be positive (or None), got %r" % (clip_grad_norm,))
        self.clip_grad_norm = None if clip_grad_norm is None else float(clip_grad_norm)
        self.grad_guard = bool(grad_guard) or self.clip_grad_norm is not None
        for name, rate in (("lr", lr), ("lr_g", lr_g), ("lr_d", lr_d)):
            if rate is not None and not float(rate) >= 0.0:
                raise ValueError("%s must not be negative, got %r" % (name, rate))
        self.per_network_lr = lr_g is not None or lr_d is not None
        lr_g, lr_d = float(lr if lr_g is None else lr_g), float(lr if lr_d is None else lr_d)
        knots = None if lr_schedule is None else _schedule.validate(lr_schedule)
        self.device = torch.device(device)
        self.aug = None
        if augment is not None:
            from . import augment as _augment
            if isinstance(augment, dict):
                rank = dist.get_rank() if dist.is_available() and dist.is_initialized() else 0
                augment = _augment.Augment(**dict({"rank": rank, "device": self.device}, **augment))
            elif not isinstance(augment, _augment.Augment):
                raise TypeError("augment: None, an augment.Augment or a dict of its arguments, got %r" % (type(augment),))
            self.aug = augment
        self.G = (generator or PointGenerator(num_k=num_k, base_points=base_points)).to(self.device)
        self.D = [d.to(self.device) for d in
                  (discriminators or [PointDiscriminator(i, (2 * base_points) << (i - 1)) for i in (1, 2, 3, 4)])]
        self.local_pair = LocalPairLoss(20)
        self.distributed = world_size() > 1 if distributed is None else distributed
        self._buckets = os.environ.get("PDGN_BUCKETS", "1") == "1"
        deepest = (list(self.G.bilateral4.parameters()) + list(self.G.mlp4.parameters())) if self._buckets and hasattr(self.G, "bilateral4") else None
        self.gradG = FlatGrads(self.G.parameters(), first=deepest)
        if self.distributed and self._buckets:
            self.gradG.arm_early()
        self.gradD = [FlatGrads(d.parameters()) for d in self.D]
        cap = self.device.type == "cuda"
        adam = lambda m, lr: torch.optim.Adam(m.parameters(), lr=lr, betas=(0.5, 0.999), capturable=cap, fused=cap and os.environ.get("PDGN_FUSED_ADAM", "1") == "1")
        self.optG, self.optD = adam(self.G, lr_g if self.per_network_lr else lr), [adam(d, lr_d if self.per_network_lr else lr) for d in self.D]
        self.lr_table = None if knots is None else _schedule.table(knots, self.device)
        self.ema_buf = self.ema = self._ema_spare = None
        if self.ema_decay > 0:
            self.ema_buf, self.ema = self._flat_like(self.optG.param_groups[0]["params"])
        self.guard_buf = self.guards = None
        if self.grad_guard:
            self.guard_buf = torch.zeros(len(self.GUARD_KEYS), GUARD_RECORD_FLOATS, dtype=torch.float32, device=self.device)
            self.guards = [GradGuard(o.param_groups[0]["params"], self.clip_grad_norm, self.guard_buf[i])
                           for i, o in enumerate([self.optG] + self.optD)]
        guard_of = lambda i: self.guards[i] if self.guards is not None else None
        self._stepG = LeanAdamStep(self.optG, self.ema, self.ema_decay, guard_of(0), self.lr_table)
        self._stepD = [LeanAdamStep(o, guard=guard_of(1 + i), sched=self.lr_table) for i, o in enumerate(self.optD)]
        self.overlap = cap and os.environ.get("PDGN_OVERLAP", "1") == "1"
        self._side = None
        self._lw = {}
        for ws in {1, world_size() if self.distributed else 1}:
            self._loss_weights(ws)
        self._early_tail = os.environ.get("PDGN_EARLY_TAIL", "1") == "1"
        self._split_d = os.environ.get("PDGN_SPLIT_D", "1") == "1"
        self._defer_d = os.environ.get("PDGN_DEFER_D", "1") == "1"
        self._ema_from_parameters()
        self.sync_replicas()

    GUARD_KEYS = ("G", "D1", "D2", "D3", "D4")

    def guard_state(self):
        if self.guards is None:
            raise RuntimeError("guard_state(): this trainer has no gradient guard (grad_guard=False, clip_grad_norm=None)")
        if self.device.type == "cuda":
            torch.cuda.synchronize(self.device)
        host = self.guard_buf.cpu()
        return {k: GradGuard.decode(host[i]) for i, k in enumerate(self.GUARD_KEYS)}

    def set_lr_schedule(self, knots):
        if self.lr_table is None:
            raise RuntimeError("set_lr_schedule(): this trainer was built without an lr_schedule; build it with one (e.g. [(0, 1.0)])")
        fresh = _schedule.table(knots, "cpu")
        with torch.no_grad():
            self.lr_table.copy_(fresh)

    def set_augment(self, **changes):
        if self.aug is None:
            raise RuntimeError("set_augment(): this trainer was built without augment; build it with one (e.g. augment={'p': 0.0})")
        self.aug.set(**changes)

    def aug_state(self):
        if self.aug is None:
            raise RuntimeError("aug_state(): this trainer was built without augment")
        return self.aug.state()

    def lr_state(self):
        if self.device.type == "cuda":
            torch.cuda.synchronize(self.device)
        tab = None if self.lr_table is None else self.lr_table.cpu()
        out = {}
        for key, opt in zip(self.GUARD_KEYS, [self.optG] + self.optD):
            g = opt.param_groups[0]
            st = opt.state.get(g["params"][0])
            step = float(st["step"]) if st and "step" in st else 0.0
            f = 1.0 if tab is None else _schedule.factor(tab, step)
            out[key] = {"step": int(step), "factor": f, "lr": float(g["lr"]) * f}
        return out

    @staticmethod
    def _flat_like(params):
        slot = lambda p: (p.numel() + 3) // 4 * 4
        buf = torch.zeros(sum(slot(p) for p in params), dtype=torch.float32, device=params[0].device)
        views, off = [], 0
        for p in params:
            views.append(buf[off:off + p.numel()].view_as(p))
            off += slot(p)
        return buf, views

    def _ema_from_parameters(self):
        if self.ema is not None:
            with torch.no_grad():
                torch._foreach_copy_(self.ema, [p.detach() for p in self.optG.param_groups[0]["params"]])

    @contextlib.contextmanager
    def averaged_generator(self):
        if self.ema is None:
            raise RuntimeError("averaged_generator(): this trainer keeps no averaged generator (ema_decay=0)")
        params = self.optG.param_groups[0]["params"]
        if self.device.type == "cuda":
            torch.cuda.synchronize(self.device)
        if self._ema_spare is None:
            self._ema_spare = self._flat_like(params)
        own = hasattr(self.G, "forward_hints")
        hints = self.G.forward_hints() if own else None
        with torch.no_grad():
            torch._foreach_copy_(self._ema_spare[1], [p.detach() for p in params])
            torch._foreach_copy_(list(params), self.ema)
        if own:
            self.G.drop_preassembled()
        try:
            yield self.G
        finally:
            with torch.no_grad():
                torch._foreach_copy_(list(params), self._ema_spare[1])
            if own:
                self.G.drop_preassembled()
                self.G.restore_forward_hints(hints)

    def sync_replicas(self, src=0):
        if not (self.distributed and dist.is_available() and dist.is_initialized() and dist.get_world_size() > 1):
            return
        with torch.no_grad():
            for net in [self.G] + self.D:
                flat = [t for t in list(net.parameters()) + list(net.buffers())]
                for dtype in sorted({t.dtype for t in flat}, key=str):
                    group = [t for t in flat if t.dtype == dtype]
                    buf = torch.cat([t.reshape(-1) for t in group])
                    dist.broadcast(buf, src)
                    off = 0
                    for t in group:
                        t.copy_(buf[off:off + t.numel()].view_as(t))
                        off += t.numel()
            for opt in [self.optG] + self.optD:
                for st in opt.state.values():
                    for v in st.values():
                        if torch.is_tensor(v):
                            dist.broadcast(v, src)
            if self.ema_buf is not None:
                dist.broadcast(self.ema_buf, src)
            if self.lr_table is not None:
                dist.broadcast(self.lr_table, src)

    def train(self):
        self.G.train()
        for d in self.D:
            d.train()

    @staticmethod
    def _ref_model_state(module):
        return {"module." + k: v.detach().cpu() for k, v in module.state_dict().items()}

    @staticmethod
    def _ref_optim_state(opt):
        sd = opt.state_dict()
        state = {}
        for i, st in sd["state"].items():
            state[i] = {k: (int(v.item()) if k == "step" else v.detach().cpu()) if torch.is_tensor(v) else v
                        for k, v in st.items()}
        keep = ("lr", "betas", "eps", "weight_decay", "amsgrad", "params")
        groups = [{k: g[k] for k in keep} for g in sd["param_groups"]]
        return {"state": state, "param_groups": groups}

    def save(self, checkpoint_dir, index_epoch, category="chair"):
        os.makedirs(checkpoint_dir, exist_ok=True)
        stem = os.path.join(checkpoint_dir, "%s_%s" % (index_epoch, category))
        held = hold_bn_counters(False)
        flush_bn_counters()
        hold_bn_counters(held)
        torch.save({"G_model": self._ref_model_state(self.G), "G_optimizer": self._ref_optim_state(self.optG),
                    "G_epoch": index_epoch}, stem + "_G.pth")
        dfile = {"D_epoch": index_epoch}
        for i, (d, o) in enumerate(zip(self.D, self.optD), 1):
            dfile["D_model%d" % i] = self._ref_model_state(d)
            dfile["D_optimizer%d" % i] = self._ref_optim_state(o)
        torch.save(dfile, stem + "_D.pth")
        if self.ema is not None:
            model = self._ref_model_state(self.G)
            for (name, p), e in zip(self.G.named_parameters(), self._ema_in_module_order()):
                assert model["module." + name].shape == e.shape, name
                model["module." + name] = e.detach().cpu().clone()
            torch.save({"G_model": model, "G_optimizer": self._ref_optim_state(self.optG), "G_epoch": index_epoch,
                        "ema_decay": self.ema_decay}, stem + "_G_ema.pth")
            return stem + "_G.pth", stem + "_D.pth", stem + "_G_ema.pth"
        return stem + "_G.pth", stem + "_D.pth"

    def _ema_in_module_order(self):
        by_id = {id(p): e for p, e in zip(self.optG.param_groups[0]["params"], self.ema)}
        return [by_id[id(p)] for p in self.G.parameters()]

    @staticmethod
    def _load_optim(opt, sd):
        groups = []
        for mine, theirs in zip(opt.state_dict()["param_groups"], sd["param_groups"]):
            g = dict(mine)
            g.update({k: theirs[k] for k in ("lr", "betas", "eps", "weight_decay", "amsgrad") if k in theirs})
            groups.append(g)
        opt.load_state_dict({"state": sd["state"], "param_groups": groups})

    def load(self, path_G, path_D):
        from .generator import load_reference_state_dict
        g = torch.load(path_G, map_location="cpu")
        d = torch.load(path_D, map_location="cpu")
        load_reference_state_dict(self.G, g["G_model"])
        self._load_optim(self.optG, g["G_optimizer"])
        for i, (m, o) in enumerate(zip(self.D, self.optD), 1):
            load_reference_state_dict(m, d["D_model%d" % i])
            self._load_optim(o, d["D_optimizer%d" % i])
        for st in [self._stepG] + self._stepD:
            st.reset()
        if self.ema is not None:
            sibling = str(path_G)[:-len("_G.pth")] + "_G_ema.pth" if str(path_G).endswith("_G.pth") else None
            if sibling is not None and os.path.exists(sibling):
                avg = torch.load(sibling, map_location="cpu")["G_model"]
                avg = {(k[len("module."):] if k.startswith("module.") else k): v for k, v in avg.items()}
                with torch.no_grad():
                    for (name, _), e in zip(self.G.named_parameters(), self._ema_in_module_order()):
                        e.copy_(avg[name])
            else:
                self._ema_from_parameters()
        self.sync_replicas()
        return g["G_epoch"]

    def _loss_weights(self, ws):
        w = self._lw.get(ws)
        if w is None:
            w = self._lw[ws] = torch.tensor([1.2, 1.2, 1.2, 1.0, 0.1 * ws], dtype=torch.float32, device=self.device)
        return w

    def _freeze_D(self, frozen):
        params = self.__dict__.get("_d_params")
        if params is None:
            params = self.__dict__["_d_params"] = [p for d in self.D for p in d.parameters()]
        for p in params:
            p.requires_grad_(not frozen)

    def similar_terms(self, clouds, pairs, own=None):
        terms, own = {}, ({} if own is None else own)
        for a, b in pairs:
            if a not in own:
                cl = clouds[a].transpose(1, 2).contiguous()
                own[a] = self.local_pair.stats(cl, cl)
            terms[(a, b)] = self.local_pair(clouds[a], clouds[b], self_stats=own[a])
        return terms

    @staticmethod
    def _sum_terms(terms):
        return torch.stack([terms[p][0] for p in PAIRS] + [terms[p][1] for p in PAIRS]).sum()

    def similar_loss(self, clouds):
        return self._sum_terms(self.similar_terms(clouds, PAIRS))

    def _seg_d(self, st, i):
        D = self.D[i]
        self.gradD[i].begin()
        if self.aug is None:
            lossD = losses.mse_const(D(st["reals"][i]), 1.0, 0.5) + losses.mse_const(D(st["fakes"][i]), 0.0, 0.5)
        else:
            lossD = (losses.mse_const(D(st["reals"][i], self.aug.at(i, "real")), 1.0, 0.5)
                     + losses.mse_const(D(st["fakes"][i], self.aug.at(i, "fake")), 0.0, 0.5))
        lossD.backward()
        st["out"]["d_loss%d" % (i + 1)] = lossD.detach()

    def _seg_d_real(self, st, i):
        D = self.D[i]
        self.gradD[i].begin()
        params = self.gradD[i].params
        loss_r = losses.mse_const(D(st["reals"][i]) if self.aug is None else D(st["reals"][i], self.aug.at(i, "real")), 1.0, 0.5)
        st["d_half"][i] = (loss_r.detach(), torch.autograd.grad(loss_r, params))

    def _seg_d_fake(self, st, i):
        D = self.D[i]
        fg = self.gradD[i]
        fg.resume()
        loss_f = losses.mse_const(D(st["fakes"][i]) if self.aug is None else D(st["fakes"][i], self.aug.at(i, "fake")), 0.0, 0.5)
        loss_r, g_real = st["d_half"][i]
        st.setdefault("keep", []).append(loss_r)
        g_fake = torch.autograd.grad(loss_f, fg.params)
        torch._foreach_add_(g_real, g_fake)
        for p, g in zip(fg.params, g_real):
            p.grad = g
        st["d_half"][i] = None
        st["out"]["d_loss%d" % (i + 1)] = loss_r + loss_f.detach()

    def _segment(self, st, k):
        if k == 0:
            if self.aug is not None:
                self.aug.tick()
            with torch.no_grad():
                st["fakes"] = self.G(self._z(st, "z1"))
            self._seg_d(st, 0)
        elif k in (1, 2, 3):
            self._stepD[k - 1].step()
            self._seg_d(st, k)
        elif k == 4:
            self._stepD[3].step()
            self.gradG.begin()
            self._freeze_D(True)
            gen = self.G(self._z(st, "z2"))
            similar = self.similar_loss(gen)
            g_loss = [losses.mse_const(self.D[i](gen[i]) if self.aug is None else self.D[i](gen[i], self.aug.at(i, "gen")), 1.0) for i in range(4)]
            adv = 1.2 * g_loss[0] + 1.2 * g_loss[1] + 1.2 * g_loss[2] + g_loss[3]
            lossG = adv + 0.1 * similar
            ws = st["ws"]
            (adv + (0.1 * ws) * similar if ws > 1 else lossG).backward()
            self._freeze_D(False)
            st["out"]["g_loss"], st["out"]["similar_loss"] = lossG.detach(), similar.detach()
        else:
            self._stepG.step()

    def _z(self, st, name):
        z = st[name]
        return z if z is not None else torch.randn(st["B"], 128, device=self.device) * 0.2

    def _comm(self, k):
        if self.distributed and k < 5:
            fg = self.gradD[k] if k < 4 else self.gradG
            fg.pack()
            fg.all_reduce_mean()

    def _state(self, reals, z1, z2):
        B = reals[0].shape[0]
        return {"reals": reals, "z1": z1, "z2": z2, "B": B, "out": {}, "ws": world_size() if self.distributed else 1}

    def step(self, reals, z1, z2):
        _warn_if_deterministic("step")
        if self.overlap:
            return self._step_overlapped(reals, z1, z2)
        st = self._state(reals, z1, z2)
        for k in range(6):
            self._segment(st, k)
            self._comm(k)
        release_zero_arena()
        return st["out"]

    def _step_overlapped(self, reals, z1, z2, st=None):
        held_counts = hold_bn_counters(True)
        try:
            return self._step_overlapped_body(reals, z1, z2, st)
        finally:
            hold_bn_counters(held_counts)
            flush_bn_counters()

    def _step_overlapped_body(self, reals, z1, z2, st=None):
        st = st if st is not None else self._state(reals, z1, z2)
        main = torch.cuda.current_stream(self.device)
        pl = _streams.plan(self.device)
        self._side, self._side_lp = pl.d, pl.lp
        st["fakes"] = [None] * 4
        st["keep"] = []
        mark = st.get("mark") or (lambda name: None)
        mark("start")
        if st.get("tag_streams"):
            from . import replay as _replay
            _replay.mark(_replay.MAIN, main)
        if self.aug is not None:
            self.aug.tick()
        if st.get("tag_streams"):
            for sid, s in enumerate(list(pl.d) + [pl.lp, pl.knn], 1):
                s.wait_stream(main)
                _replay.mark(sid, s)

        levels = []

        def d_mark(level, cloud):
            st["fakes"][level] = cloud
            ev = torch.cuda.Event()
            ev.record(torch.cuda.current_stream(self.device))
            levels.append((level, ev))
            if level < 3:
                mark("G(z1) level %d" % (level + 1))

        split = self._split_d

        def d_update(level, ev):
            side = self._side[level]
            side.wait_event(ev)
            with torch.cuda.stream(side), torch.enable_grad():
                if split:
                    self._seg_d_fake(st, level)
                else:
                    self._seg_d(st, level)
                self._comm(level)
                self._stepD[level].step()

        pre_ok = hasattr(self.G, "preassemble") and os.environ.get("PDGN_PREASM", "1") == "1"
        if pre_ok:
            with torch.enable_grad():
                self.G.preassemble(deepest_without_graph=self.distributed and self._buckets)
        if split:
            st["d_half"] = [None] * 4
            for level, side in enumerate(self._side):
                side.wait_stream(main)
                with torch.cuda.stream(side), torch.enable_grad():
                    self._seg_d_real(st, level)

        def d_now(level, cloud):
            d_mark(level, cloud)
            d_update(*levels.pop())

        hook1 = d_mark if self._defer_d else d_now
        with torch.no_grad():
            self.G(self._z(st, "z1"), stage_hook=hook1)
        for level, ev in levels:
            d_update(level, ev)
        mark("G(z1) level 4")
        self.gradG.begin()
        self._freeze_D(True)
        terms, own, g_loss, gen_so_far = {}, {}, [None] * 4, []
        early = self._early_tail

        def d_gen(level, cloud):
            side = self._side[level]
            side.wait_stream(main)
            with torch.cuda.stream(side):
                g_loss[level] = losses.mse_const(self.D[level](cloud) if self.aug is None else self.D[level](cloud, self.aug.at(level, "gen")), 1.0)

        def tail(level, cloud):
            gen_so_far.append(cloud)
            if level >= 1:
                self._side_lp.wait_stream(main)
                with torch.cuda.stream(self._side_lp):
                    terms.update(self.similar_terms(gen_so_far, [(a, level) for a in range(level)], own))
            d_gen(level, cloud)

        gen = self.G(self._z(st, "z2"), stage_hook=tail if early else None)
        mark("G(z2) forward")
        if not early:
            self._side_lp.wait_stream(main)
            with torch.cuda.stream(self._side_lp):
                terms = self.similar_terms(gen, PAIRS)
            for i, side in enumerate(self._side):
                side.wait_stream(main)
                with torch.cuda.stream(side):
                    g_loss[i] = losses.mse_const(self.D[i](gen[i]) if self.aug is None else self.D[i](gen[i], self.aug.at(i, "gen")), 1.0)
        for side in self._side:
            main.wait_stream(side)
        main.wait_stream(self._side_lp)
        mark("wait: D(gen) + local-pair forward")
        similar = self._sum_terms(terms)
        ws = st["ws"]
        terms = torch.stack(g_loss + [similar])
        lossG = (terms * self._loss_weights(1)).sum()
        (lossG if ws == 1 else (terms * self._loss_weights(ws)).sum()).backward()
        mark("backward")
        self._freeze_D(False)
        st["out"]["g_loss"], st["out"]["similar_loss"] = lossG.detach(), similar.detach()
        self._comm(4)
        self._stepG.step()
        if pre_ok:
            self.G.drop_preassembled()
        release_zero_arena()
        mark("all-reduce + Adam G")
        return st["out"]

    def capture(self, reals, z1=None, z2=None, warmup=3):
        self._static = self._state([r.clone() for r in reals], z1.clone() if z1 is not None else None,
                                   z2.clone() if z2 is not None else None)
        side = torch.cuda.Stream(device=self.device)
        side.wait_stream(torch.cuda.current_stream(self.device))
        with torch.cuda.stream(side):
            for _ in range(warmup):
                for k in range(6):
                    self._segment(self._static, k)
                    self._comm(k)
        torch.cuda.current_stream(self.device).wait_stream(side)
        torch.cuda.synchronize(self.device)
        groups = [[k] for k in range(6)] if self.distributed else [list(range(6))]
        self._graphs, pool = [], None
        if self.overlap and not self.distributed:
            g = torch.cuda.CUDAGraph()
            defer, self._defer_d = self._defer_d, False
            try:
                with torch.cuda.graph(g):
                    self._step_overlapped(None, None, None, st=self._static)
            finally:
                self._defer_d = defer
            self._graphs.append((g, 5))
            release_zero_arena()
            return self
        for group in groups:
            g = torch.cuda.CUDAGraph()
            with torch.cuda.graph(g, pool=pool, capture_error_mode="thread_local"):
                for k in group:
                    self._segment(self._static, k)
            pool = g.pool()
            self._graphs.append((g, group[-1]))
            self._comm(group[-1])
        release_zero_arena()
        return self

    def capture_list(self, reals, z1, z2, warmup=2):
        from . import replay
        if not self.overlap:
            raise RuntimeError("capture_list: stream-overlapped schedule only")
        _warn_if_deterministic("capture_list")
        self._static = self._state([r.clone() for r in reals], z1.clone(), z2.clone())
        side = torch.cuda.Stream(device=self.device)
        side.wait_stream(torch.cuda.current_stream(self.device))
        with torch.cuda.stream(side):
            for _ in range(warmup):
                self._step_overlapped(None, None, None, st=self._state(self._static["reals"], self._static["z1"], self._static["z2"]))
        torch.cuda.current_stream(self.device).wait_stream(side)
        torch.cuda.synchronize(self.device)
        if self.distributed and dist.is_available() and dist.is_initialized():
            for fg in (self.gradG, *self.gradD):
                if getattr(fg, "_early_work", None) is not None:
                    fg._early_work.wait()
                    fg._early_work = None
            import time
            time.sleep(float(os.environ.get("PDGN_CAPTURE_QUIESCE_S", "0.5")))
        g = torch.cuda.CUDAGraph(keep_graph=True)
        defer, self._defer_d = self._defer_d, False
        self._static["tag_streams"] = True
        rec = replay.Recorder()
        try:
            with rec, torch.cuda.graph(g, capture_error_mode="thread_local"):
                self._step_overlapped(None, None, None, st=self._static)
        finally:
            self._defer_d = defer
            self._static.pop("tag_streams", None)
        release_zero_arena()
        self._list = replay.LaunchList(g)
        if len(self._list.points) != len(rec.fns):
            raise RuntimeError("capture_list: %d host points recorded, %d found in the list" % (len(rec.fns), len(self._list.points)))
        self._list_points = [(pos, rec.fns[i], label) for pos, i, label in self._list.points]
        info = self._list.info
        if info["chains"] != info["labelled"] or not self._list.joined:
            raise RuntimeError("capture_list: %d chains, %d tagged, joined=%s: a launch on an untagged stream, or a side stream whose "
                               "last launch the issuing stream never waits for" % (info["chains"], info["labelled"], self._list.joined))
        self._list_spare = [torch.cuda.Stream(device=self.device) for _ in range(2)]
        self._list_done = None
        self._list_pace = float(os.environ.get("PDGN_LIST_PACE", "1.0"))
        return self

    def step_list(self, reals=None, z1=None, z2=None):
        from . import replay
        st = self._static
        if reals is not None:
            for d, s in zip(st["reals"], reals):
                if d.data_ptr() != s.data_ptr():
                    d.copy_(s)
        if z1 is not None:
            st["z1"].copy_(z1)
            st["z2"].copy_(z2)
        pl = _streams.plan(self.device)
        streams = {replay.MAIN: torch.cuda.current_stream(self.device), replay.LP: pl.lp, replay.KNN: pl.knn}
        for i, s in enumerate(pl.d):
            streams[replay.D0 + i] = s
        self._list.bind(streams, self._list_spare)
        if self._list_done is not None:
            self._list_done.synchronize()
        cut = self._list.position(replay.MAIN, self._list_pace)
        stops = sorted([(cut, 0, None, None)] + [(pos + 1, 1, fn, label) for pos, fn, label in self._list_points], key=lambda t: t[:2])
        lo = 0
        for at, kind, fn, label in stops:
            if at > lo:
                self._list.launch(lo, at)
                lo = at
            if kind == 0:
                if self._list_done is None:
                    self._list_done = torch.cuda.Event()
                self._list_done.record(streams[replay.MAIN])
            else:
                with torch.cuda.stream(streams[label]):
                    fn()
        self._list.launch(lo)
        return st["out"]

    LOG_FORMAT = ("Epoch: [%2d] [%4d/%4d] time: %2dm %2ds d_loss1: %.8f d_loss2: %.8f d_loss3: %.8f d_loss4: %.8f, "
                  "g_loss: %.8f, similar_loss: %.8f")
    LOSS_KEYS = ("d_loss1", "d_loss2", "d_loss3", "d_loss4", "g_loss", "similar_loss")

    def fit(self, feeder, epochs, start_epoch=1, snapshot=20, checkpoint_dir=None, category="chair", issue="list", log=None,
            on_epoch=None, guard_max_skips=50, grad_norms=None, lr_log=None):
        import time
        if issue not in ("list", "eager"):
            raise ValueError("issue: 'list' or 'eager', got %r" % (issue,))
        guarded = getattr(self, "guards", None) is not None
        if guarded and int(guard_max_skips) < 1:
            raise ValueError("guard_max_skips must be at least one, got %r" % (guard_max_skips,))
        sink, opened = log, None
        if isinstance(log, (str, bytes, os.PathLike)):
            opened = open(log, "a")
            sink = lambda line: (opened.write(line + "\n"), opened.flush())
        nb = feeder.batches_per_epoch
        cuda = self.device.type == "cuda"
        nl, nk = len(self.LOSS_KEYS), len(PDGNTrainer.GUARD_KEYS)
        host = torch.empty(2, nl + (nk * GUARD_RECORD_FLOATS if guarded else 0), dtype=torch.float32, pin_memory=cuda)
        done = [torch.cuda.Event() for _ in range(2)] if cuda else None
        pending, n, start = None, 0, time.time()
        norms_file = None
        if guarded:
            if grad_norms is None and isinstance(log, (str, bytes, os.PathLike)):
                grad_norms = os.path.join(os.path.dirname(os.fspath(log)) or ".", "grad_norms.csv")
            if grad_norms is not None and getattr(feeder, "rank", 0) == 0:
                fresh = not os.path.exists(grad_norms) or os.path.getsize(grad_norms) == 0
                norms_file = open(grad_norms, "a")
                if fresh:
                    norms_file.write(",".join(["epoch", "iter"] + ["%s_%s" % (k, f) for k in PDGNTrainer.GUARD_KEYS for f in ("norm", "coef")]
                                              + ["skipped_total"]) + "\n")
            skipped_before, run_of_skips = None, [0] * nk
        rates_file, rates_epoch = None, None
        if getattr(self, "lr_table", None) is not None or getattr(self, "per_network_lr", False):
            if lr_log is None and isinstance(log, (str, bytes, os.PathLike)):
                lr_log = os.path.join(os.path.dirname(os.fspath(log)) or ".", "lr.csv")
            if lr_log is not None and getattr(feeder, "rank", 0) == 0:
                fresh = not os.path.exists(lr_log) or os.path.getsize(lr_log) == 0
                rates_file = open(lr_log, "a")
                if fresh:
                    rates_file.write(",".join(["epoch", "step_G"] + ["lr_%s" % k for k in PDGNTrainer.GUARD_KEYS]) + "\n")

        def rates_line(ep):
            nonlocal rates_epoch
            if rates_file is None or rates_epoch == ep:
                return
            rates_epoch = ep
            state = self.lr_state()
            rates_file.write(",".join(["%d" % ep, "%d" % state["G"]["step"]] + ["%.17g" % state[k]["lr"] for k in PDGNTrainer.GUARD_KEYS]) + "\n")
            rates_file.flush()

        def flush():
            slot, ep, idx = pending
            if cuda:
                done[slot].synchronize()
            dt = time.time() - start
            if sink is not None:
                sink(self.LOG_FORMAT % ((ep, idx + 1, nb, dt / 60, dt % 60) + tuple(host[slot, :nl].tolist())))
            if guarded:
                guard_line(ep, idx, [GradGuard.decode(host[slot, nl + i * GUARD_RECORD_FLOATS:nl + (i + 1) * GUARD_RECORD_FLOATS]) for i in range(nk)])

        def guard_line(ep, idx, recs):
            nonlocal skipped_before
            if norms_file is not None:
                norms_file.write(",".join(["%d" % ep, "%d" % (idx + 1)] + ["%.9g" % r[f] for r in recs for f in ("norm", "coef")]
                                          + ["%d" % sum(r["skipped"] for r in recs)]) + "\n")
                norms_file.flush()
            now = [r["skipped"] for r in recs]
            if skipped_before is not None:
                for i in range(nk):
                    run_of_skips[i] = run_of_skips[i] + 1 if now[i] != skipped_before[i] else 0
            else:
                for i in range(nk):
                    run_of_skips[i] = 1 if recs[i]["applied"] + recs[i]["skipped"] > 0 and PDGNTrainer._last_skipped(recs[i]) else 0
            skipped_before = now
            worst = max(range(nk), key=lambda i: run_of_skips[i])
            if run_of_skips[worst] >= int(guard_max_skips):
                where = ""
                if checkpoint_dir is not None and getattr(feeder, "rank", 0) == 0:
                    where = "; checkpoint of the last finite parameters: " + self.save(checkpoint_dir, ep, category)[0]
                raise GradGuardError("gradient guard: %s skipped %d consecutive updates (epoch %d, iteration %d): its gradients are "
                                     "not finite%s" % (PDGNTrainer.GUARD_KEYS[worst], run_of_skips[worst], ep, idx + 1, where))

        try:
            if issue == "eager" or getattr(self, "_list", None) is None:
                reals, z1, z2 = feeder.buffers()
            if issue == "list" and getattr(self, "_list", None) is None and start_epoch <= epochs:
                feeder.fill(start_epoch, 0, reals, z1, z2)
                self.capture_list(reals, z1, z2)
            if issue == "list":
                st = self._static
                reals, z1, z2 = st["reals"], st["z1"], st["z2"]
            if getattr(self, "aug", None) is not None:
                self.aug.set_clock((start_epoch - 1) * nb)
            for epoch in range(start_epoch, epochs + 1):
                for i in range(nb):
                    feeder.fill(epoch, i, reals, z1, z2)
                    out = self.step_list() if issue == "list" else self.step(reals, z1, z2)
                    if sink is not None or guarded:
                        slot = n & 1
                        row = torch.stack([out[k] for k in self.LOSS_KEYS])
                        host[slot].copy_(torch.cat([row, self.guard_buf.view(-1)]) if guarded else row, non_blocking=True)
                        if cuda:
                            done[slot].record(torch.cuda.current_stream(self.device))
                        if pending is not None:
                            flush()
                        pending = (slot, epoch, i)
                        n += 1
                        if guarded and max(run_of_skips) >= int(guard_max_skips) - 1:
                            flush()
                            pending = None
                if checkpoint_dir is not None and epoch % snapshot == 0 and getattr(feeder, "rank", 0) == 0:
                    self.save(checkpoint_dir, epoch, category)
                    rates_line(epoch)
                if on_epoch is not None:
                    on_epoch(epoch)
                    rates_line(epoch)
            if pending is not None:
                flush()
            if checkpoint_dir is not None and getattr(feeder, "rank", 0) == 0:
                self.save(checkpoint_dir, epochs, category)
                rates_line(epochs)
        finally:
            if opened is not None:
                opened.close()
            if norms_file is not None:
                norms_file.close()
            if rates_file is not None:
                rates_file.close()
        return epochs

    @staticmethod
    def _last_skipped(rec):
        return not (rec["norm"] == rec["norm"] and abs(rec["norm"]) != float("inf"))

    def _sync(self):
        torch.cuda.current_stream(self.device).synchronize()

    def step_graphed(self, reals=None, z1=None, z2=None):
        st = self._static
        copies = []
        if reals is not None:
            copies += [(d, s) for d, s in zip(st["reals"], reals) if d.data_ptr() != s.data_ptr()]
        if z1 is not None and st["z1"] is not None:
            copies += [(st["z1"], z1), (st["z2"], z2)]
        if copies:
            self._sync()
            for d, s in copies:
                d.copy_(s)
            self._sync()
        for g, last in self._graphs:
            g.replay()
            if self.distributed and last < 5:
                self._sync()
                fg = self.gradD[last] if last < 4 else self.gradG
                fg._early_work, fg._early_done = None, False
                self._comm(last)
                self._sync()
        return st["out"]


def synthetic_batch(B, device, seed=9999, n_points=2048, resolutions=(256, 512, 1024, 2048)):
    g = torch.Generator().manual_seed(seed)
    pts = torch.randn(B, n_points, 3, generator=g)
    pts = (pts - pts.mean(dim=1, keepdim=True)) / pts.reshape(B, -1).std(dim=1).view(B, 1, 1)
    reals = []
    for r in resolutions:
        if r == n_points:
            sub = pts
        else:
            sel = torch.randint(0, n_points, (B, r), generator=g)
            sub = torch.gather(pts, 1, sel.unsqueeze(2).expand(B, r, 3))
        reals.append(sub.transpose(1, 2).contiguous().to(device))
    return reals


def noise(B, device, generator=None):
    return (torch.randn(B, 128, generator=generator) * 0.2).to(device)
```

Measured before the change: 3.119 million points/s.

## Batch local-pair KNN, stats and chamfer terms into segmented multi-pair launches

Adds segmented kernels that run KNN queries, local mean/covariance stats, and their backward for several query clouds against one reference cloud in a single launch. Chamfer gram forward/backward and scaled sums are also batched across pairs through pointer tables. The trainer groups the similarity-loss pairs by target cloud to cut kernel launch count and Python overhead. In exchange the backward adds an extra LDS fold buffer and per-segment syncs, and enlarges the launch argument structs.

```diff
diff --git a/include/pdgn_hip.h b/include/pdgn_hip.h
--- a/include/pdgn_hip.h
+++ b/include/pdgn_hip.h
@@ -12,7 +12,7 @@
 
 typedef void *pdgn_stream_t;
 
-#define PDGN_ABI_VERSION 34
+#define PDGN_ABI_VERSION 35
 int pdgn_abi_version(void);
 
 int pdgn_knnquery(int b, int n, int m, int nsample, const float *xyz, const float *new_xyz,
@@ -214,6 +214,47 @@
 int pdgn_mse_const_backward(long long n, const float *x, float target, float scale, const float *g, float *dx,
                             pdgn_stream_t stream);
 
+#define PDGN_SEG_MAX 4
+#define PDGN_PAIR_MAX 3
+#define PDGN_SUM_MAX 8
+typedef struct pdgn_knn_segment {
+    const float *queries;
+    int32_t *idx;
+    float *dist2;
+    int m;
+} pdgn_knn_segment;
+int pdgn_knnquery_segments(int b, int n, int nsample, const float *xyz, int nseg, const pdgn_knn_segment *segs,
+                           pdgn_stream_t stream);
+typedef struct pdgn_stats_segment {
+    const int32_t *idx;
+    float *mu;
+    float *cov;
+    int m;
+} pdgn_stats_segment;
+int pdgn_local_stats_segments(int b, int n, int k, const float *xyz, int nseg, const pdgn_stats_segment *segs,
+                              pdgn_stream_t stream);
+int pdgn_local_stats_backward_segments(int b, int n, int k, const float *xyz, int nseg, const pdgn_stats_segment *segs,
+                                       float *dxyz, pdgn_stream_t stream);
+typedef struct pdgn_chamfer_pair {
+    const float *x;
+    const float *y;
+    float *mins;
+    int32_t *args;
+    const float *g;
+    float *grads;
+    int m, n;
+    float scale;
+} pdgn_chamfer_pair;
+int pdgn_chamfer_gram_pairs(int b, int d, int npairs, const pdgn_chamfer_pair *pairs, pdgn_stream_t stream);
+int pdgn_chamfer_gram_grad_pairs(int b, int d, int npairs, const pdgn_chamfer_pair *pairs, pdgn_stream_t stream);
+typedef struct pdgn_sum_term {
+    const float *x;
+    float *out;
+    long long n;
+    float scale;
+} pdgn_sum_term;
+int pdgn_scaled_sum_multi(int nterms, const pdgn_sum_term *terms, pdgn_stream_t stream);
+
 int pdgn_emd_cost_indexed(int npairs, int n, int m, const float *xyz1, const int32_t *ia,
                           const float *xyz2, const int32_t *ib, float *temp, float *out,
                           pdgn_stream_t stream);
diff --git a/pdgn_amd/csrc/knn3.hip b/pdgn_amd/csrc/knn3.hip
--- a/pdgn_amd/csrc/knn3.hip
+++ b/pdgn_amd/csrc/knn3.hip
@@ -26,10 +26,29 @@
     return __uint_as_float(ub & 0x7fffffffu);
 }
 
+struct KnnSegs {
+    const float *q[PDGN_SEG_MAX];
+    int32_t *idx[PDGN_SEG_MAX];
+    float *dist2[PDGN_SEG_MAX];
+    int m[PDGN_SEG_MAX];
+    int tile0[PDGN_SEG_MAX];
+    int nseg;
+};
+
 __global__ __launch_bounds__(KNN4_THREADS) void knn3_wave4_kernel(
-    int n, int m, int K, int qpw, const float *__restrict__ xyz, const float *__restrict__ new_xyz,
-    int32_t *__restrict__ idx, float *__restrict__ dist2) {
+    int n, int K, int qpw, const float *__restrict__ xyz, const KnnSegs segs) {
     __shared__ float4 cand[KNN4_TILE];
+    const float *__restrict__ new_xyz = segs.q[0];
+    int32_t *__restrict__ idx = segs.idx[0];
+    float *__restrict__ dist2 = segs.dist2[0];
+    int m = segs.m[0], tile0 = 0;
+#pragma unroll
+    for (int s = 1; s < PDGN_SEG_MAX; ++s)
+        if (s < segs.nseg && (int)blockIdx.x >= segs.tile0[s]) {
+            new_xyz = segs.q[s]; idx = segs.idx[s]; dist2 = segs.dist2[s];
+            m = segs.m[s]; tile0 = segs.tile0[s];
+        }
+    const int tile = (int)blockIdx.x - tile0;
     __shared__ DI queue[KNN4_WAVES][KNN4_Q][KNN4_QCAP + KNN_FAST_MAX_K];
     __shared__ DI win[KNN4_WAVES][KNN4_Q][KNN_FAST_MAX_K];
 
@@ -38,7 +57,7 @@
     const int wave = threadIdx.x / PDGN_WAVE;
     const float *P = xyz + (size_t)bs * n * 3;
   for (int grp = 0; grp < qpw; ++grp) {
-    const int q0 = ((blockIdx.x * KNN4_WAVES + wave) * qpw + grp) * KNN4_Q;
+    const int q0 = ((tile * KNN4_WAVES + wave) * qpw + grp) * KNN4_Q;
 
     float qx[KNN4_Q], qy[KNN4_Q], qz[KNN4_Q], rd[KNN4_Q];
     int ri[KNN4_Q], cnt[KNN4_Q];
@@ -247,22 +266,46 @@
     }
 }
 
+extern "C" int pdgn_knnquery_segments(int b, int n, int nsample, const float *xyz, int nseg, const pdgn_knn_segment *segs,
+                                      pdgn_stream_t stream) {
+    if (b < 0 || n < 0 || nsample < 1 || nsample > PDGN_KNN_MAX_NSAMPLE || nseg < 0 || nseg > PDGN_SEG_MAX || (nseg && !segs))
+        return PDGN_ERR_INVALID;
+    for (int s = 0; s < nseg; ++s)
+        if (segs[s].m < 0 || (segs[s].m && (!segs[s].queries || !segs[s].idx))) return PDGN_ERR_INVALID;
+    if (b == 0) return 0;
+    if (b > 65535) return PDGN_ERR_INVALID;
+    hipStream_t st = (hipStream_t)stream;
+    if (nsample <= KNN_FAST_MAX_K) {
+        KnnSegs a = {};
+        int tiles = 0;
+        for (int s = 0; s < nseg; ++s) {
+            if (segs[s].m == 0) continue;
+            a.q[a.nseg] = segs[s].queries; a.idx[a.nseg] = segs[s].idx; a.dist2[a.nseg] = segs[s].dist2;
+            a.m[a.nseg] = segs[s].m; a.tile0[a.nseg] = tiles;
+            tiles += cdiv(segs[s].m, KNN4_WAVES * KNN4_Q);
+            ++a.nseg;
+        }
+        if (a.nseg == 0) return 0;
+        hipLaunchKernelGGL(knn3_wave4_kernel, dim3(tiles, b), dim3(KNN4_THREADS), 0, st, n, nsample, 1, xyz, a);
+        return pdgn_launch_status();
+    }
+    for (int s = 0; s < nseg; ++s) {
+        if (segs[s].m == 0) continue;
+        hipLaunchKernelGGL(knn3_generic_kernel, dim3(cdiv(segs[s].m, KNN_THREADS), b), dim3(KNN_THREADS), 0, st, n, segs[s].m,
+                           nsample, xyz, segs[s].queries, segs[s].idx, segs[s].dist2);
+        const int rc = pdgn_launch_status();
+        if (rc) return rc;
+    }
+    return 0;
+}
+
 extern "C" int pdgn_knnquery(int b, int n, int m, int nsample, const float *xyz,
                              const float *new_xyz, int32_t *idx, float *dist2,
                              pdgn_stream_t stream) {
     if (b < 0 || n < 0 || m < 0 || nsample < 1 || nsample > PDGN_KNN_MAX_NSAMPLE) return PDGN_ERR_INVALID;
     if (b == 0 || m == 0) return 0;
-    if (b > 65535) return PDGN_ERR_INVALID;
-    hipStream_t s = (hipStream_t)stream;
-    if (nsample <= KNN_FAST_MAX_K) {
-        dim3 grid(cdiv(m, KNN4_WAVES * KNN4_Q), b);
-        hipLaunchKernelGGL(knn3_wave4_kernel, grid, dim3(KNN4_THREADS), 0, s, n, m, nsample, 1, xyz, new_xyz, idx, dist2);
-    } else {
-        dim3 grid(cdiv(m, KNN_THREADS), b);
-        hipLaunchKernelGGL(knn3_generic_kernel, grid, dim3(KNN_THREADS), 0, s, n, m, nsample, xyz,
-                           new_xyz, idx, dist2);
-    }
-    return pdgn_launch_status();
+    const pdgn_knn_segment one = {new_xyz, idx, dist2, m};
+    return pdgn_knnquery_segments(b, n, nsample, xyz, 1, &one, stream);
 }
 
 extern "C" int pdgn_nearestneighbor(int b, int n, int m, const float *unknown, const float *known,
diff --git a/pdgn_amd/csrc/localpair.hip b/pdgn_amd/csrc/localpair.hip
--- a/pdgn_amd/csrc/localpair.hip
+++ b/pdgn_amd/csrc/localpair.hip
@@ -5,11 +5,30 @@
 #define LP_LDS_FLOATS 8192
 #define LP_PTS_FLOATS 6144
 
+struct StatSegs {
+    const int32_t *idx[PDGN_SEG_MAX];
+    float *mu[PDGN_SEG_MAX];
+    float *cov[PDGN_SEG_MAX];
+    int m[PDGN_SEG_MAX];
+    int tile0[PDGN_SEG_MAX];
+    int qsplit[PDGN_SEG_MAX];
+    int nseg;
+};
+
 __global__ __launch_bounds__(LP_THREADS) void local_stats_fwd_kernel(
-    int n, int m, int K, const float *__restrict__ xyz, const int32_t *__restrict__ idx,
-    float *__restrict__ mu, float *__restrict__ cov) {
+    int n, int K, const float *__restrict__ xyz, const StatSegs segs) {
+    const int32_t *__restrict__ idx = segs.idx[0];
+    float *__restrict__ mu = segs.mu[0];
+    float *__restrict__ cov = segs.cov[0];
+    int m = segs.m[0], tile0 = 0;
+#pragma unroll
+    for (int s = 1; s < PDGN_SEG_MAX; ++s)
+        if (s < segs.nseg && (int)blockIdx.x >= segs.tile0[s]) {
+            idx = segs.idx[s]; mu = segs.mu[s]; cov = segs.cov[s];
+            m = segs.m[s]; tile0 = segs.tile0[s];
+        }
     const int bs = blockIdx.y;
-    const int q = blockIdx.x * blockDim.x + threadIdx.x;
+    const int q = ((int)blockIdx.x - tile0) * blockDim.x + threadIdx.x;
     if (q >= m) return;
     const float *P = xyz + (size_t)bs * n * 3;
     const int32_t *I = idx + ((size_t)bs * m + q) * K;
@@ -36,12 +55,13 @@
 }
 
 __global__ __launch_bounds__(LP_THREADS) void local_stats_bwd_kernel(
-    int n, int m, int K, int qsplit, const float *__restrict__ xyz, const int32_t *__restrict__ idx,
-    const float *__restrict__ dmu, const float *__restrict__ dcov, float *__restrict__ dxyz) {
+    int n, int K, const float *__restrict__ xyz, const StatSegs segs, float *__restrict__ dxyz) {
     __shared__ float slab[LP_LDS_FLOATS];
+    __shared__ float total[LP_LDS_FLOATS];
     __shared__ float pts[LP_PTS_FLOATS];
     const int bs = blockIdx.y;
     const bool use_lds = n * 3 <= LP_LDS_FLOATS, use_pts = n * 3 <= LP_PTS_FLOATS;
+    const bool fold = use_lds && segs.nseg > 1;
     const float *P = xyz + (size_t)bs * n * 3;
     if (use_lds)
         for (int i = threadIdx.x; i < n * 3; i += LP_THREADS) slab[i] = 0.f;
@@ -50,9 +70,17 @@
     if (use_lds || use_pts) __syncthreads();
     auto pt = [&](int j, int c) { return use_pts ? pts[j * 3 + c] : P[(size_t)j * 3 + c]; };
     float *D = dxyz + (size_t)bs * n * 3;
+    const float invK = 1.0f / (float)K;
+#pragma unroll 1
+  for (int sg = 0; sg < segs.nseg; ++sg) {
+    if (sg > 0) __syncthreads();
+    const int m = segs.m[sg], qsplit = segs.qsplit[sg];
+    const int32_t *__restrict__ idx = segs.idx[sg];
+    const float *__restrict__ dmu = segs.mu[sg];
+    const float *__restrict__ dcov = segs.cov[sg];
     const int per = (m + qsplit - 1) / qsplit;
-    const int q0 = blockIdx.x * per, q1 = min(m, q0 + per);
-    const float invK = 1.0f / (float)K;
+    const int q0 = blockIdx.x * per;
+    const int q1 = (int)blockIdx.x < qsplit ? min(m, q0 + per) : 0;
     for (int q = q0 + threadIdx.x; q < q1; q += LP_THREADS) {
         const int32_t *I = idx + ((size_t)bs * m + q) * K;
         float sx = 0.f, sy = 0.f, sz = 0.f;
@@ -76,10 +104,19 @@
             atomicAdd(dst, gx); atomicAdd(dst + 1, gy); atomicAdd(dst + 2, gz);
         }
     }
+    if (fold) {
+        __syncthreads();
+        for (int i = threadIdx.x; i < n * 3; i += LP_THREADS) {
+            const float v = slab[i];
+            total[i] = sg == 0 ? v : total[i] + v;
+            slab[i] = 0.f;
+        }
+    }
+  }
     if (use_lds) {
         __syncthreads();
         for (int i = threadIdx.x; i < n * 3; i += LP_THREADS) {
-            float v = slab[i];
+            float v = fold ? total[i] : slab[i];
             if (v != 0.f) atomicAdd(&D[i], v);
         }
     }
@@ -88,15 +125,38 @@
 #define CH_MAXD 16
 #define CH_TILE 1024
 
+struct ChPairs {
+    const float *x[PDGN_PAIR_MAX];
+    const float *y[PDGN_PAIR_MAX];
+    float *minx[PDGN_PAIR_MAX];
+    int32_t *argx[PDGN_PAIR_MAX];
+    float *miny[PDGN_PAIR_MAX];
+    int32_t *argy[PDGN_PAIR_MAX];
+    int m[PDGN_PAIR_MAX];
+    int n[PDGN_PAIR_MAX];
+};
+
 template <int D>
 __global__ __launch_bounds__(LP_THREADS) void chamfer_gram_kernel(
-    int m, int n, int dd, const float *__restrict__ x, const float *__restrict__ y,
-    float *__restrict__ minx, int32_t *__restrict__ argx, float *__restrict__ miny,
-    int32_t *__restrict__ argy, const int32_t *__restrict__ ia, const int32_t *__restrict__ ib) {
+    int b, int dd, const ChPairs tab, const int32_t *__restrict__ ia, const int32_t *__restrict__ ib) {
     constexpr int DS = D > 0 ? D : CH_MAXD;
     __shared__ float cand[CH_TILE * (DS + 1)];
     const int d = D > 0 ? D : dd;
-    const int bs = blockIdx.y;
+    const int pr = blockIdx.y / b;
+    const int bs = blockIdx.y - pr * b;
+    const float *__restrict__ x = tab.x[0];
+    const float *__restrict__ y = tab.y[0];
+    float *__restrict__ minx = tab.minx[0];
+    float *__restrict__ miny = tab.miny[0];
+    int32_t *__restrict__ argx = tab.argx[0];
+    int32_t *__restrict__ argy = tab.argy[0];
+    int m = tab.m[0], n = tab.n[0];
+#pragma unroll
+    for (int p = 1; p < PDGN_PAIR_MAX; ++p)
+        if (pr == p) {
+            x = tab.x[p]; y = tab.y[p]; minx = tab.minx[p]; miny = tab.miny[p]; argx = tab.argx[p]; argy = tab.argy[p];
+            m = tab.m[p]; n = tab.n[p];
+        }
     const bool rev = blockIdx.z != 0;
     const int nq = rev ? n : m, nc = rev ? m : n;
     if ((int)(blockIdx.x * blockDim.x) >= nq) return;
@@ -168,14 +228,41 @@
 
 #define CHL_THREADS 1024
 #define CHL_MAXF 12288
+struct ChGradPairs {
+    const float *x[PDGN_PAIR_MAX];
+    const float *y[PDGN_PAIR_MAX];
+    const int32_t *argx[PDGN_PAIR_MAX];
+    const int32_t *argy[PDGN_PAIR_MAX];
+    float *gx[PDGN_PAIR_MAX];
+    float *gy[PDGN_PAIR_MAX];
+    const float *guni[PDGN_PAIR_MAX];
+    int m[PDGN_PAIR_MAX];
+    int n[PDGN_PAIR_MAX];
+    float gscale[PDGN_PAIR_MAX];
+};
+
 template <int D>
 __global__ __launch_bounds__(CHL_THREADS) void chamfer_gram_grad_lds_kernel(
-    int m, int n, int d, const float *__restrict__ x, const float *__restrict__ y,
-    const float *__restrict__ gminx, const int32_t *__restrict__ argx, const float *__restrict__ gminy,
-    const int32_t *__restrict__ argy, float *__restrict__ gx, float *__restrict__ gy, const float *__restrict__ guni, float gscale) {
+    int b, int d, const ChGradPairs tab, const float *__restrict__ gminx, const float *__restrict__ gminy) {
     __shared__ float accs[CHL_MAXF];
     const int dd = D > 0 ? D : d;
-    const int bs = blockIdx.y;
+    const int pr = blockIdx.y / b;
+    const int bs = blockIdx.y - pr * b;
+    const float *__restrict__ x = tab.x[0];
+    const float *__restrict__ y = tab.y[0];
+    const int32_t *__restrict__ argx = tab.argx[0];
+    const int32_t *__restrict__ argy = tab.argy[0];
+    float *__restrict__ gx = tab.gx[0];
+    float *__restrict__ gy = tab.gy[0];
+    const float *__restrict__ guni = tab.guni[0];
+    int m = tab.m[0], n = tab.n[0];
+    float gscale = tab.gscale[0];
+#pragma unroll
+    for (int p = 1; p < PDGN_PAIR_MAX; ++p)
+        if (pr == p) {
+            x = tab.x[p]; y = tab.y[p]; argx = tab.argx[p]; argy = tab.argy[p]; gx = tab.gx[p]; gy = tab.gy[p];
+            guni = tab.guni[p]; m = tab.m[p]; n = tab.n[p]; gscale = tab.gscale[p];
+        }
     const bool rev = blockIdx.z != 0;
     const int nq = rev ? n : m, nc = rev ? m : n;
     const float *Qb = (rev ? y : x) + (size_t)bs * nq * dd, *Cb = (rev ? x : y) + (size_t)bs * nc * dd;
@@ -200,13 +287,54 @@
     for (int f = threadIdx.x; f < nq * dd; f += CHL_THREADS) G[f] = accs[f];
 }
 
+static int stats_table(int b, int nseg, const pdgn_stats_segment *segs, StatSegs *a, int *tiles, int *max_split) {
+    if (nseg < 0 || nseg > PDGN_SEG_MAX || (nseg && !segs)) return PDGN_ERR_INVALID;
+    *a = StatSegs{};
+    *tiles = *max_split = 0;
+    for (int s = 0; s < nseg; ++s) {
+        const int m = segs[s].m;
+        if (m < 0 || (m && (!segs[s].idx || !segs[s].mu || !segs[s].cov))) return PDGN_ERR_INVALID;
+        if (m == 0) continue;
+        int qsplit = b > 0 ? 1024 / b : 1;
+        const int ms = cdiv(m, LP_THREADS);
+        qsplit = qsplit < 1 ? 1 : (qsplit > ms ? ms : qsplit);
+        const int k = a->nseg++;
+        a->idx[k] = segs[s].idx; a->mu[k] = segs[s].mu; a->cov[k] = segs[s].cov;
+        a->m[k] = m; a->tile0[k] = *tiles; a->qsplit[k] = qsplit;
+        *tiles += ms;
+        *max_split = qsplit > *max_split ? qsplit : *max_split;
+    }
+    return 0;
+}
+
+extern "C" int pdgn_local_stats_segments(int b, int n, int k, const float *xyz, int nseg, const pdgn_stats_segment *segs,
+                                         pdgn_stream_t stream) {
+    if (b < 0 || n < 1 || k < 1 || b > 65535) return PDGN_ERR_INVALID;
+    StatSegs a;
+    int tiles, max_split;
+    if (stats_table(b, nseg, segs, &a, &tiles, &max_split)) return PDGN_ERR_INVALID;
+    if (b == 0 || a.nseg == 0) return 0;
+    hipLaunchKernelGGL(local_stats_fwd_kernel, dim3(tiles, b), dim3(LP_THREADS), 0, (hipStream_t)stream, n, k, xyz, a);
+    return pdgn_launch_status();
+}
+
+extern "C" int pdgn_local_stats_backward_segments(int b, int n, int k, const float *xyz, int nseg,
+                                                  const pdgn_stats_segment *segs, float *dxyz, pdgn_stream_t stream) {
+    if (b < 0 || n < 1 || k < 1 || b > 65535) return PDGN_ERR_INVALID;
+    StatSegs a;
+    int tiles, max_split;
+    if (stats_table(b, nseg, segs, &a, &tiles, &max_split)) return PDGN_ERR_INVALID;
+    if (b == 0 || a.nseg == 0) return 0;
+    hipLaunchKernelGGL(local_stats_bwd_kernel, dim3(max_split, b), dim3(LP_THREADS), 0, (hipStream_t)stream, n, k, xyz, a, dxyz);
+    return pdgn_launch_status();
+}
+
 extern "C" int pdgn_local_stats(int b, int n, int m, int k, const float *xyz, const int32_t *idx, float *mu,
                                 float *cov, pdgn_stream_t stream) {
     if (b < 0 || n < 1 || m < 0 || k < 1 || b > 65535) return PDGN_ERR_INVALID;
     if (b == 0 || m == 0) return 0;
-    hipLaunchKernelGGL(local_stats_fwd_kernel, dim3(cdiv(m, LP_THREADS), b), dim3(LP_THREADS), 0,
-                       (hipStream_t)stream, n, m, k, xyz, idx, mu, cov);
-    return pdgn_launch_status();
+    const pdgn_stats_segment one = {idx, mu, cov, m};
+    return pdgn_local_stats_segments(b, n, k, xyz, 1, &one, stream);
 }
 
 extern "C" int pdgn_local_stats_backward(int b, int n, int m, int k, const float *xyz, const int32_t *idx,
@@ -214,23 +342,42 @@
                                          pdgn_stream_t stream) {
     if (b < 0 || n < 1 || m < 0 || k < 1 || b > 65535) return PDGN_ERR_INVALID;
     if (b == 0 || m == 0) return 0;
-    int qsplit = 1024 / b;
-    const int max_split = cdiv(m, LP_THREADS);
-    qsplit = qsplit < 1 ? 1 : (qsplit > max_split ? max_split : qsplit);
-    hipLaunchKernelGGL(local_stats_bwd_kernel, dim3(qsplit, b), dim3(LP_THREADS), 0, (hipStream_t)stream, n, m, k,
-                       qsplit, xyz, idx, dmu, dcov, dxyz);
+    const pdgn_stats_segment one = {idx, const_cast<float *>(dmu), const_cast<float *>(dcov), m};
+    return pdgn_local_stats_backward_segments(b, n, k, xyz, 1, &one, dxyz, stream);
+}
+
+static int chamfer_launch(dim3 grid, hipStream_t s, int b, int d, const ChPairs &tab, const int32_t *ia, const int32_t *ib) {
+    if (d == 3)
+        hipLaunchKernelGGL(chamfer_gram_kernel<3>, grid, dim3(LP_THREADS), 0, s, b, d, tab, ia, ib);
+    else if (d == 9)
+        hipLaunchKernelGGL(chamfer_gram_kernel<9>, grid, dim3(LP_THREADS), 0, s, b, d, tab, ia, ib);
+    else
+        hipLaunchKernelGGL(chamfer_gram_kernel<0>, grid, dim3(LP_THREADS), 0, s, b, d, tab, ia, ib);
     return pdgn_launch_status();
 }
 
-static int chamfer_launch(dim3 grid, hipStream_t s, int m, int n, int d, const float *x, const float *y, float *minx,
-                          int32_t *argx, float *miny, int32_t *argy, const int32_t *ia, const int32_t *ib) {
-    if (d == 3)
-        hipLaunchKernelGGL(chamfer_gram_kernel<3>, grid, dim3(LP_THREADS), 0, s, m, n, d, x, y, minx, argx, miny, argy, ia, ib);
-    else if (d == 9)
-        hipLaunchKernelGGL(chamfer_gram_kernel<9>, grid, dim3(LP_THREADS), 0, s, m, n, d, x, y, minx, argx, miny, argy, ia, ib);
-    else
-        hipLaunchKernelGGL(chamfer_gram_kernel<0>, grid, dim3(LP_THREADS), 0, s, m, n, d, x, y, minx, argx, miny, argy, ia, ib);
-    return pdgn_launch_status();
+static ChPairs one_pair(int m, int n, const float *x, const float *y, float *minx, int32_t *argx, float *miny, int32_t *argy) {
+    ChPairs t = {};
+    t.x[0] = x; t.y[0] = y; t.minx[0] = minx; t.argx[0] = argx; t.miny[0] = miny; t.argy[0] = argy; t.m[0] = m; t.n[0] = n;
+    return t;
+}
+
+extern "C" int pdgn_chamfer_gram_pairs(int b, int d, int npairs, const pdgn_chamfer_pair *pairs, pdgn_stream_t stream) {
+    if (b < 0 || d < 1 || d > CH_MAXD || npairs < 0 || npairs > PDGN_PAIR_MAX || (npairs && !pairs) || (long long)b * npairs > 65535)
+        return PDGN_ERR_INVALID;
+    ChPairs t = {};
+    int big = 0;
+    for (int p = 0; p < npairs; ++p) {
+        const pdgn_chamfer_pair &e = pairs[p];
+        if (e.m < 1 || e.n < 1 || !e.x || !e.y || !e.mins || !e.args) return PDGN_ERR_INVALID;
+        t.x[p] = e.x; t.y[p] = e.y; t.m[p] = e.m; t.n[p] = e.n;
+        t.minx[p] = e.mins; t.miny[p] = e.mins + (size_t)b * e.m;
+        t.argx[p] = e.args; t.argy[p] = e.args + (size_t)b * e.m;
+        big = e.m > big ? e.m : big;
+        big = e.n > big ? e.n : big;
+    }
+    if (b == 0 || npairs == 0) return 0;
+    return chamfer_launch(dim3(cdiv(big, LP_THREADS), b * npairs, 2), (hipStream_t)stream, b, d, t, nullptr, nullptr);
 }
 
 extern "C" int pdgn_chamfer_gram(int b, int m, int n, int d, const float *x, const float *y, float *minx,
@@ -238,8 +385,7 @@
     if (b < 0 || m < 1 || n < 1 || d < 1 || d > CH_MAXD || b > 65535) return PDGN_ERR_INVALID;
     if (b == 0) return 0;
     dim3 grid(cdiv(m > n ? m : n, LP_THREADS), b, 2);
-    hipStream_t s = (hipStream_t)stream;
-    return chamfer_launch(grid, s, m, n, d, x, y, minx, argx, miny, argy, nullptr, nullptr);
+    return chamfer_launch(grid, (hipStream_t)stream, b, d, one_pair(m, n, x, y, minx, argx, miny, argy), nullptr, nullptr);
 }
 
 extern "C" int pdgn_chamfer_gram_indexed(int npairs, int m, int n, int d, const float *x, const int32_t *ia,
@@ -248,7 +394,23 @@
     if (npairs < 0 || m < 1 || n < 1 || d < 1 || d > CH_MAXD || npairs > 65535) return PDGN_ERR_INVALID;
     if (npairs == 0) return 0;
     dim3 grid(cdiv(m > n ? m : n, LP_THREADS), npairs, 2);
-    return chamfer_launch(grid, (hipStream_t)stream, m, n, d, x, y, minx, argx, miny, argy, ia, ib);
+    return chamfer_launch(grid, (hipStream_t)stream, npairs, d, one_pair(m, n, x, y, minx, argx, miny, argy), ia, ib);
+}
+
+static bool chamfer_in_lds() {
+    static const bool in_lds = !(getenv("PDGN_CHAMFER_LDS") && getenv("PDGN_CHAMFER_LDS")[0] == '0');
+    return in_lds;
+}
+
+static int chamfer_grad_lds_launch(int b, int d, int npairs, const ChGradPairs &t, const float *gminx, const float *gminy, hipStream_t s) {
+    dim3 grid(1, b * npairs, 2);
+    if (d == 3)
+        hipLaunchKernelGGL(chamfer_gram_grad_lds_kernel<3>, grid, dim3(CHL_THREADS), 0, s, b, d, t, gminx, gminy);
+    else if (d == 9)
+        hipLaunchKernelGGL(chamfer_gram_grad_lds_kernel<9>, grid, dim3(CHL_THREADS), 0, s, b, d, t, gminx, gminy);
+    else
+        hipLaunchKernelGGL(chamfer_gram_grad_lds_kernel<0>, grid, dim3(CHL_THREADS), 0, s, b, d, t, gminx, gminy);
+    return pdgn_launch_status();
 }
 
 static int chamfer_grad_launch(int b, int m, int n, int d, const float *x, const float *y, const float *gminx, const int32_t *argx,
@@ -256,19 +418,11 @@
                                hipStream_t s) {
     hipError_t e;
     const size_t nx = (size_t)b * m * d, ny = (size_t)b * n * d;
-    static const bool in_lds = !(getenv("PDGN_CHAMFER_LDS") && getenv("PDGN_CHAMFER_LDS")[0] == '0');
-    if (in_lds && (size_t)m * d <= CHL_MAXF && (size_t)n * d <= CHL_MAXF) {
-        dim3 grid(1, b, 2);
-        if (d == 3)
-            hipLaunchKernelGGL(chamfer_gram_grad_lds_kernel<3>, grid, dim3(CHL_THREADS), 0, s, m, n, d, x, y, gminx, argx, gminy, argy,
-                               gx, gy, guni, gscale);
-        else if (d == 9)
-            hipLaunchKernelGGL(chamfer_gram_grad_lds_kernel<9>, grid, dim3(CHL_THREADS), 0, s, m, n, d, x, y, gminx, argx, gminy, argy,
-                               gx, gy, guni, gscale);
-        else
-            hipLaunchKernelGGL(chamfer_gram_grad_lds_kernel<0>, grid, dim3(CHL_THREADS), 0, s, m, n, d, x, y, gminx, argx, gminy, argy,
-                               gx, gy, guni, gscale);
-        return pdgn_launch_status();
+    if (chamfer_in_lds() && (size_t)m * d <= CHL_MAXF && (size_t)n * d <= CHL_MAXF) {
+        ChGradPairs t = {};
+        t.x[0] = x; t.y[0] = y; t.argx[0] = argx; t.argy[0] = argy; t.gx[0] = gx; t.gy[0] = gy; t.guni[0] = guni;
+        t.m[0] = m; t.n[0] = n; t.gscale[0] = gscale;
+        return chamfer_grad_lds_launch(b, d, 1, t, gminx, gminy, s);
     }
     if (gy == gx + nx) {
         if ((e = hipMemsetAsync(gx, 0, (nx + ny) * sizeof(float), s)) != hipSuccess) return (int)e;
@@ -297,3 +451,26 @@
     if (b == 0) return 0;
     return chamfer_grad_launch(b, m, n, d, x, y, nullptr, argx, nullptr, argy, gx, gy, g, scale, (hipStream_t)stream);
 }
+
+extern "C" int pdgn_chamfer_gram_grad_pairs(int b, int d, int npairs, const pdgn_chamfer_pair *pairs, pdgn_stream_t stream) {
+    if (b < 0 || d < 1 || d > CH_MAXD || npairs < 0 || npairs > PDGN_PAIR_MAX || (npairs && !pairs) || (long long)b * npairs > 65535)
+        return PDGN_ERR_INVALID;
+    ChGradPairs t = {};
+    bool fits = chamfer_in_lds();
+    for (int p = 0; p < npairs; ++p) {
+        const pdgn_chamfer_pair &e = pairs[p];
+        if (e.m < 1 || e.n < 1 || !e.x || !e.y || !e.args || !e.g || !e.grads) return PDGN_ERR_INVALID;
+        t.x[p] = e.x; t.y[p] = e.y; t.m[p] = e.m; t.n[p] = e.n; t.guni[p] = e.g; t.gscale[p] = e.scale;
+        t.argx[p] = e.args; t.argy[p] = e.args + (size_t)b * e.m;
+        t.gx[p] = e.grads; t.gy[p] = e.grads + (size_t)b * e.m * d;
+        fits = fits && (size_t)e.m * d <= CHL_MAXF && (size_t)e.n * d <= CHL_MAXF;
+    }
+    if (b == 0 || npairs == 0) return 0;
+    if (fits) return chamfer_grad_lds_launch(b, d, npairs, t, nullptr, nullptr, (hipStream_t)stream);
+    for (int p = 0; p < npairs; ++p) {
+        const int rc = chamfer_grad_launch(b, t.m[p], t.n[p], d, t.x[p], t.y[p], nullptr, t.argx[p], nullptr, t.argy[p], t.gx[p],
+                                           t.gy[p], t.guni[p], t.gscale[p], (hipStream_t)stream);
+        if (rc) return rc;
+    }
+    return 0;
+}
diff --git a/pdgn_amd/csrc/loss_small.hip b/pdgn_amd/csrc/loss_small.hip
--- a/pdgn_amd/csrc/loss_small.hip
+++ b/pdgn_amd/csrc/loss_small.hip
@@ -14,8 +14,21 @@
     return s;
 }
 
-__global__ __launch_bounds__(LS_THREADS) void scaled_sum_kernel(long long n, const float *__restrict__ x, float scale,
-                                                               float *__restrict__ out) {
+struct SumTerms {
+    const float *x[PDGN_SUM_MAX];
+    float *out[PDGN_SUM_MAX];
+    long long n[PDGN_SUM_MAX];
+    float scale[PDGN_SUM_MAX];
+};
+
+__global__ __launch_bounds__(LS_THREADS) void scaled_sum_kernel(const SumTerms tab) {
+    const float *__restrict__ x = tab.x[0];
+    float *__restrict__ out = tab.out[0];
+    long long n = tab.n[0];
+    float scale = tab.scale[0];
+#pragma unroll
+    for (int t = 1; t < PDGN_SUM_MAX; ++t)
+        if ((int)blockIdx.x == t) { x = tab.x[t]; out = tab.out[t]; n = tab.n[t]; scale = tab.scale[t]; }
     float s = 0.f;
     for (long long i = threadIdx.x; i < n; i += LS_THREADS) s += x[i];
     s = ls_block_sum(s);
@@ -40,10 +53,22 @@
         dx[i] = c * (x[i] - t);
 }
 
+extern "C" int pdgn_scaled_sum_multi(int nterms, const pdgn_sum_term *terms, pdgn_stream_t stream) {
+    if (nterms < 0 || nterms > PDGN_SUM_MAX || (nterms && !terms)) return PDGN_ERR_INVALID;
+    SumTerms t = {};
+    for (int i = 0; i < nterms; ++i) {
+        if (terms[i].n < 0 || !terms[i].out || (terms[i].n && !terms[i].x)) return PDGN_ERR_INVALID;
+        t.x[i] = terms[i].x; t.out[i] = terms[i].out; t.n[i] = terms[i].n; t.scale[i] = terms[i].scale;
+    }
+    if (nterms == 0) return 0;
+    hipLaunchKernelGGL(scaled_sum_kernel, dim3(nterms), dim3(LS_THREADS), 0, (hipStream_t)stream, t);
+    return pdgn_launch_status();
+}
+
 extern "C" int pdgn_scaled_sum(long long n, const float *x, float scale, float *out, pdgn_stream_t stream) {
     if (n < 0) return PDGN_ERR_INVALID;
-    hipLaunchKernelGGL(scaled_sum_kernel, dim3(1), dim3(LS_THREADS), 0, (hipStream_t)stream, n, x, scale, out);
-    return pdgn_launch_status();
+    const pdgn_sum_term one = {x, out, n, scale};
+    return pdgn_scaled_sum_multi(1, &one, stream);
 }
 
 extern "C" int pdgn_mse_const(long long n, const float *x, float target, float scale, float *out, pdgn_stream_t stream) {
diff --git a/pdgn_amd/losses.py b/pdgn_amd/losses.py
--- a/pdgn_amd/losses.py
+++ b/pdgn_amd/losses.py
@@ -1,3 +1,6 @@
+
+import ctypes
+import os
 
 import torch
 import torch.nn as nn
@@ -8,6 +11,52 @@
 from .fused import _zeros
 
 F32, I32 = torch.float32, torch.int32
+
+PAIR_BATCH = os.environ.get("PDGN_PAIR_BATCH", "1") == "1"
+SEG_MAX, PAIR_MAX, SUM_MAX = 4, 3, 8
+
+
+class KnnSegment(ctypes.Structure):
+    _fields_ = [("queries", ctypes.c_void_p), ("idx", ctypes.c_void_p), ("dist2", ctypes.c_void_p), ("m", ctypes.c_int)]
+
+
+class StatsSegment(ctypes.Structure):
+    _fields_ = [("idx", ctypes.c_void_p), ("mu", ctypes.c_void_p), ("cov", ctypes.c_void_p), ("m", ctypes.c_int)]
+
+
+class ChamferPair(ctypes.Structure):
+    _fields_ = [("x", ctypes.c_void_p), ("y", ctypes.c_void_p), ("mins", ctypes.c_void_p), ("args", ctypes.c_void_p),
+                ("g", ctypes.c_void_p), ("grads", ctypes.c_void_p), ("m", ctypes.c_int), ("n", ctypes.c_int),
+                ("scale", ctypes.c_float)]
+
+
+class SumTerm(ctypes.Structure):
+    _fields_ = [("x", ctypes.c_void_p), ("out", ctypes.c_void_p), ("n", ctypes.c_longlong), ("scale", ctypes.c_float)]
+
+
+def pack_table(struct, rows, limit):
+    rows = list(rows)
+    if not 1 <= len(rows) <= limit:
+        raise ValueError("%s table: %d entries, 1 .. %d are supported" % (struct.__name__, len(rows), limit))
+    width = len(struct._fields_)
+    for r in rows:
+        if len(r) != width:
+            raise ValueError("%s entry: %d values for %d fields" % (struct.__name__, len(r), width))
+    return (struct * len(rows))(*[struct(*r) for r in rows])
+
+
+def chunks(seq, size):
+    seq = list(seq)
+    return [seq[i:i + size] for i in range(0, len(seq), size)]
+
+
+def _carve(buf, counts, shapes=None):
+    out, off = [], 0
+    for i, c in enumerate(counts):
+        v = buf[off:off + c]
+        out.append(v if shapes is None else v.view(shapes[i]))
+        off += c
+    return out
 
 
 class ChamferGram(Function):
@@ -141,6 +190,117 @@
     return LocalStats.apply(xyz, idx)
 
 
+class SegmentStats(Function):
+
+    @staticmethod
+    def forward(ctx, nsample, xyz, *queries):
+        require(xyz, "xyz", F32, 3)
+        b, n, _ = xyz.shape
+        for q in queries:
+            require(q, "queries", F32, 3)
+            if q.shape[0] != b or q.shape[2] != 3:
+                raise ValueError("queries must be (%d, m, 3), got %s" % (b, tuple(q.shape)))
+        if xyz.shape[2] != 3:
+            raise ValueError("xyz must be (B, N, 3), got %s" % (tuple(xyz.shape),))
+        ms = [int(q.shape[1]) for q in queries]
+        k = int(nsample)
+        idx = _carve(torch.empty((b * sum(ms) * k,), dtype=I32, device=xyz.device), [b * m * k for m in ms],
+                     [(b, m, k) for m in ms])
+        stats = _carve(torch.empty((b * sum(ms) * 12,), dtype=F32, device=xyz.device), [c for m in ms for c in (b * m * 3, b * m * 9)],
+                       [sh for m in ms for sh in ((b, m, 3), (b, m, 9))])
+        L, st = _lib.lib(), stream_of(xyz)
+        knn = pack_table(KnnSegment, [(q.data_ptr(), i.data_ptr(), None, m) for q, i, m in zip(queries, idx, ms)], SEG_MAX)
+        check(L.pdgn_knnquery_segments(b, n, k, ptr(xyz), len(ms), knn, st), "pdgn_knnquery_segments")
+        seg = pack_table(StatsSegment, [(i.data_ptr(), stats[2 * s].data_ptr(), stats[2 * s + 1].data_ptr(), m)
+                                        for s, (i, m) in enumerate(zip(idx, ms))], SEG_MAX)
+        check(L.pdgn_local_stats_segments(b, n, k, ptr(xyz), len(ms), seg, st), "pdgn_local_stats_segments")
+        ctx.save_for_backward(xyz, *idx)
+        ctx.k = k
+        return tuple(stats)
+
+    @staticmethod
+    def backward(ctx, *grads):
+        xyz, idx = ctx.saved_tensors[0], ctx.saved_tensors[1:]
+        b, n, _ = xyz.shape
+        rows, keep = [], []
+        for s, i in enumerate(idx):
+            m = i.shape[1]
+            dmu, dcov = grads[2 * s], grads[2 * s + 1]
+            dmu = torch.zeros((b, m, 3), dtype=F32, device=xyz.device) if dmu is None else dmu.contiguous()
+            dcov = torch.zeros((b, m, 9), dtype=F32, device=xyz.device) if dcov is None else dcov.contiguous()
+            keep += [dmu, dcov]
+            rows.append((i.data_ptr(), dmu.data_ptr(), dcov.data_ptr(), m))
+        dxyz = _zeros(tuple(xyz.shape), xyz.device)
+        check(_lib.lib().pdgn_local_stats_backward_segments(b, n, ctx.k, ptr(xyz), len(rows), pack_table(StatsSegment, rows, SEG_MAX),
+                                                            ptr(dxyz), stream_of(xyz)), "pdgn_local_stats_backward_segments")
+        return (None, dxyz) + (None,) * len(idx)
+
+
+def segment_stats(nsample, xyz, queries):
+    out = SegmentStats.apply(int(nsample), xyz, *queries)
+    return [(out[2 * s], out[2 * s + 1]) for s in range(len(queries))]
+
+
+class ChamferSumPairs(Function):
+
+    @staticmethod
+    def forward(ctx, *args):
+        if not args or len(args) % 3:
+            raise ValueError("ChamferSumPairs takes (x, y, scale) triples")
+        xs, ys, scales = [a.contiguous() for a in args[0::3]], [a.contiguous() for a in args[1::3]], [float(a) for a in args[2::3]]
+        b, dev = xs[0].shape[0], xs[0].device
+        for x, y in zip(xs, ys):
+            require(x, "x", F32, 3)
+            require(y, "y", F32, 3)
+            if x.shape[0] != b or y.shape[0] != b or x.shape[2] != y.shape[2]:
+                raise ValueError("a pair must be x (B, M, D), y (B, N, D) with one B for all pairs")
+        counts = [b * (x.shape[1] + y.shape[1]) for x, y in zip(xs, ys)]
+        mins = _carve(torch.empty((sum(counts),), dtype=F32, device=dev), counts)
+        amin = _carve(torch.empty((sum(counts),), dtype=I32, device=dev), counts)
+        outs = torch.empty((len(xs),), dtype=F32, device=dev)
+        L, st = _lib.lib(), stream_of(xs[0])
+        for d, members in ChamferSumPairs._by_dim(xs):
+            for run in chunks(members, PAIR_MAX):
+                tab = pack_table(ChamferPair, [(xs[i].data_ptr(), ys[i].data_ptr(), mins[i].data_ptr(), amin[i].data_ptr(), None, None,
+                                                xs[i].shape[1], ys[i].shape[1], scales[i]) for i in run], PAIR_MAX)
+                check(L.pdgn_chamfer_gram_pairs(b, d, len(run), tab, st), "pdgn_chamfer_gram_pairs")
+        for run in chunks(range(len(xs)), SUM_MAX):
+            tab = pack_table(SumTerm, [(mins[i].data_ptr(), outs[i].data_ptr(), counts[i], scales[i]) for i in run], SUM_MAX)
+            check(L.pdgn_scaled_sum_multi(len(run), tab, st), "pdgn_scaled_sum_multi")
+        ctx.save_for_backward(*xs, *ys, *amin)
+        ctx.scales = scales
+        return tuple(outs.unbind(0))
+
+    @staticmethod
+    def _by_dim(xs):
+        dims = {}
+        for i, x in enumerate(xs):
+            dims.setdefault(int(x.shape[2]), []).append(i)
+        return sorted(dims.items())
+
+    @staticmethod
+    def backward(ctx, *gs):
+        np_ = len(ctx.scales)
+        saved = ctx.saved_tensors
+        xs, ys, amin = saved[:np_], saved[np_:2 * np_], saved[2 * np_:]
+        b, dev = xs[0].shape[0], xs[0].device
+        gs = [torch.zeros((), dtype=F32, device=dev) if g is None else g.contiguous() for g in gs]
+        counts = [c for x, y in zip(xs, ys) for c in (x.numel(), y.numel())]
+        grads = _carve(torch.empty((sum(counts),), dtype=F32, device=dev), counts, [t.shape for x, y in zip(xs, ys) for t in (x, y)])
+        L, st = _lib.lib(), stream_of(xs[0])
+        for d, members in ChamferSumPairs._by_dim(xs):
+            for run in chunks(members, PAIR_MAX):
+                tab = pack_table(ChamferPair, [(xs[i].data_ptr(), ys[i].data_ptr(), None, amin[i].data_ptr(), gs[i].data_ptr(),
+                                                grads[2 * i].data_ptr(), xs[i].shape[1], ys[i].shape[1], ctx.scales[i]) for i in run],
+                                 PAIR_MAX)
+                check(L.pdgn_chamfer_gram_grad_pairs(b, d, len(run), tab, st), "pdgn_chamfer_gram_grad_pairs")
+        return tuple(v for i in range(np_) for v in (grads[2 * i], grads[2 * i + 1], None))
+
+
+def chamfer_sum_pairs(triples):
+    return list(ChamferSumPairs.apply(*[v for t in triples for v in t]))
+
+
 def knnquery(nsample, xyz, new_xyz):
     return pointops.knnquery(nsample, xyz, new_xyz)
 
@@ -174,3 +334,24 @@
         mu1, var1 = self_stats if self_stats is not None else self.stats(new_xyz, new_xyz)
         mu2, var2 = self.stats(pt2.transpose(1, 2).contiguous(), new_xyz)
         return chamfer_sum(mu2, mu1, 1.0 / float(M)), chamfer_sum(var2, var1, 1.0 / float(M))
+
+    def level(self, clouds, heads, b, own):
+        def cl(i):
+            if ("cl", i) not in own:
+                own[("cl", i)] = clouds[i].transpose(1, 2).contiguous()
+            return own[("cl", i)]
+
+        terms = {}
+        for run in chunks(heads, PAIR_MAX):
+            for a in run:
+                if a not in own:
+                    own[a] = self.stats(cl(a), cl(a))
+            around = segment_stats(self.nsample, cl(b), [cl(a) for a in run])
+            triples = []
+            for a, (mu2, var2) in zip(run, around):
+                scale = 1.0 / float(clouds[a].shape[2])
+                triples += [(mu2, own[a][0], scale), (var2, own[a][1], scale)]
+            sums = chamfer_sum_pairs(triples)
+            for i, a in enumerate(run):
+                terms[(a, b)] = (sums[2 * i], sums[2 * i + 1])
+        return terms
diff --git a/pdgn_amd/trainer.py b/pdgn_amd/trainer.py
--- a/pdgn_amd/trainer.py
+++ b/pdgn_amd/trainer.py
@@ -707,6 +707,13 @@
 
     def similar_terms(self, clouds, pairs, own=None):
         terms, own = {}, ({} if own is None else own)
+        if losses.PAIR_BATCH and clouds[0].is_cuda and not _lib.deterministic():
+            levels = {}
+            for a, b in pairs:
+                levels.setdefault(b, []).append(a)
+            for b, heads in levels.items():
+                terms.update(self.local_pair.level(clouds, heads, b, own))
+            return terms
         for a, b in pairs:
             if a not in own:
                 cl = clouds[a].transpose(1, 2).contiguous()
```

Measured after the change: 3.086 million points/s. 1.1% lower.
